# kwea123/nerf_pl

Measured on AMD Instinct MI355X. Metric: rays/sec (64+128 samples), full training step: render_rays fwd + MSE + bwd + grad all-reduce + Adam, higher is better.
Workload: dtype bf16

## Files before the change

include/nerfhip.h:

```cpp
#ifndef NERFHIP_H
#define NERFHIP_H

#include <stddef.h>
#include <stdint.h>

#ifdef __cplusplus
extern "C" {
#endif

#define NERFHIP_ABI_VERSION 3

#define NERFHIP_E_BADARG (-1)
#define NERFHIP_E_UNSUPPORTED (-2)
#define NERFHIP_E_ALIGN (-3)
#define NERFHIP_E_DATA (-4)

#define NERFHIP_F32 0
#define NERFHIP_BF16 1
#define NERFHIP_BF16_F8 2

typedef void* nerfhip_stream_t;

int nerfhip_abi_version(void);
const char* nerfhip_error_string(int code);

int nerfhip_posenc(const float* x, float* out, int64_t n, int C, int n_freqs, nerfhip_stream_t stream);
int nerfhip_posenc_bwd(const float* x, const float* gout, float* gx, int64_t n, int C, int n_freqs,
                       nerfhip_stream_t stream);

int nerfhip_posenc_bands(const float* x, const float* bands, float* out, int64_t n, int C, int n_freqs,
                         nerfhip_stream_t stream);
int nerfhip_posenc_bands_bwd(const float* x, const float* bands, const float* gout, float* gx, int64_t n, int C, int n_freqs,
                             nerfhip_stream_t stream);

int nerfhip_sample_coarse_z(const float* rays, const float* perturb_rand, float* z, int64_t B, int S,
                            int use_disp, float perturb, nerfhip_stream_t stream);

int nerfhip_searchsorted_right(const float* a, const float* v, int64_t* idx, int64_t B, int M, int K,
                               nerfhip_stream_t stream);
int nerfhip_searchsorted_left(const float* a, const float* v, int64_t* idx, int64_t B, int M, int K,
                              nerfhip_stream_t stream);

int nerfhip_sample_pdf(const float* bins, int64_t bins_stride, const float* weights, int64_t w_stride,
                       const float* u, int64_t u_stride, float* samples, int64_t B, int M, int K, float eps,
                       nerfhip_stream_t stream);

#define NERFHIP_ROW_TOTAL_EXACT 0
#define NERFHIP_ROW_TOTAL_ATEN 1

int nerfhip_sample_pdf_ex(const float* bins, int64_t bins_stride, const float* weights, int64_t w_stride,
                          const float* u, int64_t u_stride, float* samples, int64_t B, int M, int K, float eps,
                          float* cdf_out, int64_t* inds_out, int row_total, nerfhip_stream_t stream);

int nerfhip_fine_z(const float* z_coarse, const float* w_coarse, const float* u, int64_t u_stride,
                   float* z_fine, float* z_new, int64_t B, int S_c, int N_i, float eps,
                   nerfhip_stream_t stream);

int nerfhip_fine_z_ex(const float* z_coarse, const float* w_coarse, const float* u, int64_t u_stride, float* z_fine,
                      float* z_new, int64_t B, int S_c, int N_i, float eps, float* cdf_out, int64_t* inds_out,
                      int row_total, nerfhip_stream_t stream);

int nerfhip_composite_fwd(const float* raw, int raw_ch, const float* z, const float* rays,
                          const float* noise, float noise_std, int white_back, float* weights, float* rgb,
                          float* depth, float* opacity, int64_t B, int S, nerfhip_stream_t stream);
int nerfhip_composite_bwd(const float* raw, int raw_ch, const float* z, const float* rays,
                          const float* noise, float noise_std, int white_back, const float* g_rgb,
                          const float* g_depth, const float* g_opacity, const float* g_weights,
                          float* g_raw, int64_t B, int S, nerfhip_stream_t stream);

int nerfhip_composite_train(const float* raw, const float* z, const float* rays, const float* noise, float noise_std,
                            int white_back, const float* target, float grad_scale, float* weights, float* rgb, float* depth,
                            float* opacity, float* g_raw, int64_t B, int S, nerfhip_stream_t stream);

int nerfhip_composite_train_fine_z(const float* raw, const float* z, const float* rays, const float* noise, float noise_std,
                                   int white_back, const float* target, float grad_scale, float* weights, float* rgb, float* depth,
                                   float* opacity, float* g_raw, int64_t B, int S, const float* u, int64_t u_stride, int N_i,
                                   float eps, float* z_fine, int row_total, nerfhip_stream_t stream);
int nerfhip_composite_train_loss(const float* raw, const float* z, const float* rays, const float* noise, float noise_std,
                                 int white_back, const float* target, float grad_scale, float* weights, float* rgb, float* depth,
                                 float* opacity, float* g_raw, int64_t B, int S, const float* rgb_coarse, float* out3,
                                 uint32_t* ticket, nerfhip_stream_t stream);

size_t nerfhip_mlp_packed_bytes(int dtype);
int nerfhip_mlp_pack_weights(const float* const* weights_host, const float* const* biases_host, void* packed,
                             int dtype, nerfhip_stream_t stream);

size_t nerfhip_mlp_act_bytes(int64_t n_points, int dtype);

int nerfhip_mlp_fwd_embedded(const float* x, int64_t x_stride, int64_t n, const void* packed, float* out,
                             int sigma_only, int dtype, void* save_acts, nerfhip_stream_t stream);

int nerfhip_mlp_fwd_rays(const float* rays, const float* z, int64_t B, int S, const void* packed, float* out,
                         int sigma_only, int dtype, void* save_acts, nerfhip_stream_t stream);

int nerfhip_mlp_fwd_rays_coarse(const float* rays, const float* perturb_rand, float* z, int64_t B, int S, int use_disp,
                                float perturb, const void* packed, float* out, int sigma_only, int dtype, void* save_acts,
                                nerfhip_stream_t stream);

size_t nerfhip_mlp_packed_bwd_bytes(int dtype);
int nerfhip_mlp_pack_weights_bwd(const float* const* weights_host, const float* const* biases_host, void* packed_bwd, int dtype,
                                 nerfhip_stream_t stream);
int nerfhip_mlp_pack_weights_train(const float* const* weights_host, const float* const* biases_host, void* packed,
                                   void* packed_bwd, int dtype, nerfhip_stream_t stream);
int nerfhip_mlp_pack_weights_train_multi(const float* const* weights_host, const float* const* biases_host,
                                         void* const* packed_host, void* const* packed_bwd_host, int n_models, int dtype,
                                         nerfhip_stream_t stream);
size_t nerfhip_mlp_dy_bytes(int64_t n_points, int dtype);
int nerfhip_mlp_dw_splits(int64_t n_points, int dtype);
size_t nerfhip_mlp_dw_workspace_bytes(int64_t n_points, int dtype);
int nerfhip_mlp_bwd(const float* g_out, const float* out, int64_t n, const void* packed_bwd, const void* acts,
                    void* dys, void* dw_workspace, float* const* grad_w_host, float* const* grad_b_host,
                    int accumulate, int dtype, nerfhip_stream_t stream);

int nerfhip_mlp_bwd_phases(const float* g_out, const float* out, int64_t n, const void* packed_bwd, const void* acts,
                           void* dys, void* dw_workspace, float* const* grad_w_host, float* const* grad_b_host,
                           int accumulate, int dtype, int phases, nerfhip_stream_t stream);

typedef struct nerfhip_adam_fused {
    int n_models;
    float* param[2];
    float* exp_avg[2];
    float* exp_avg_sq[2];
    const float* grad_flat[2];
    float* state;
    float lr, beta1, beta2, eps, weight_decay;
} nerfhip_adam_fused;
size_t nerfhip_mlp_dw_workspace_bytes_multi(const int64_t* n_points_host, int n_models, int dtype);
int nerfhip_mlp_dw_plan(const int64_t* n_points_host, int n_models, int dtype, int* splits_out, int* stage_kib_out);
int nerfhip_mlp_bwd_multi(int n_models, const float* const* g_out_host, const float* const* out_host, const int64_t* n_host,
                          const void* const* packed_bwd_host, const void* const* acts_host, void* const* dys_host,
                          void* dw_workspace, float* const* grad_w_host, float* const* grad_b_host, int accumulate, int dtype,
                          int phases, const float* g_scale, const nerfhip_adam_fused* adam, nerfhip_stream_t stream);

typedef struct nerfhip_enc_source {
    const float* rays[2];
    const float* z[2];
    int S[2];
} nerfhip_enc_source;
int nerfhip_mlp_bwd_multi_rays(int n_models, const float* const* g_out_host, const float* const* out_host, const int64_t* n_host,
                               const void* const* packed_bwd_host, const void* const* acts_host, void* const* dys_host,
                               void* dw_workspace, float* const* grad_w_host, float* const* grad_b_host, int accumulate, int dtype,
                               int phases, const float* g_scale, const nerfhip_adam_fused* adam, const nerfhip_enc_source* enc,
                               nerfhip_stream_t stream);

int nerfhip_mlp_dx_embedded(const void* dys, int64_t n, const float* w_xyz1, const float* w_xyz5, const float* w_dir,
                            float* gx, int64_t gx_stride, int dtype, nerfhip_stream_t stream);

#define NERFHIP_ACT_NONE 0
#define NERFHIP_ACT_RELU 1
#define NERFHIP_ACT_SIGMOID 2
int nerfhip_linear_fwd(const float* x, int64_t ldx, const float* w, int64_t ldw, const float* bias, float* y, int64_t ldy,
                       int64_t n, int n_in, int n_out, int act, int accumulate, int dtype, nerfhip_stream_t stream);
int nerfhip_linear_bwd_input(const float* gy, int64_t ldgy, const float* y, int64_t ldy, int act, const float* w, int64_t ldw,
                             float* gx, int64_t ldgx, int64_t n, int n_in, int n_out, int accumulate, int dtype,
                             nerfhip_stream_t stream);
size_t nerfhip_linear_bwd_weight_workspace_bytes(int64_t n, int n_in, int n_out);
int nerfhip_linear_bwd_weight(const float* gy, int64_t ldgy, const float* y, int64_t ldy, int act, const float* x, int64_t ldx,
                              float* gw, int64_t ldgw, float* gb, void* workspace, int64_t n, int n_in, int n_out,
                              int accumulate, int dtype, nerfhip_stream_t stream);

int nerfhip_mse_psnr(const float* rgb_coarse, const float* rgb_fine, const float* target, int64_t n, float* out3,
                     float* g_coarse, float* g_fine, nerfhip_stream_t stream);

int nerfhip_adam_step(float* const* params_host, const float* const* grads_host, float* const* exp_avg_host,
                      float* const* exp_avg_sq_host, const int64_t* numel_host, int n_tensors, float* state, float lr,
                      float beta1, float beta2, float eps, float weight_decay, nerfhip_stream_t stream);

int nerfhip_radam_step(float* const* params_host, const float* const* grads_host, float* const* exp_avg_host,
                       float* const* exp_avg_sq_host, const int64_t* numel_host, int n_tensors, float* state, double lr,
                       double beta1, double beta2, double eps, double weight_decay, int degenerated_to_sgd,
                       nerfhip_stream_t stream);
int nerfhip_ranger_step(float* const* params_host, const float* const* grads_host, float* const* exp_avg_host,
                        float* const* exp_avg_sq_host, const int64_t* numel_host, int n_tensors, float* state,
                        float* const* slow_host, double alpha, int k, double n_sma_threshold, double lr, double beta1,
                        double beta2, double eps, double weight_decay, nerfhip_stream_t stream);

int nerfhip_ray_directions(float* dirs, int H, int W, double focal, nerfhip_stream_t stream);
int nerfhip_get_rays(const float* directions, const float* c2w, float* rays_o, float* rays_d, int64_t n,
                     nerfhip_stream_t stream);
int nerfhip_ndc_rays(int H, int W, double focal, float near, const float* rays_o, const float* rays_d, float* out_o,
                     float* out_d, int64_t n, nerfhip_stream_t stream);
int nerfhip_gen_rays(const float* c2w, const int64_t* pixel_ids, int64_t first_pixel, int64_t n, int H, int W,
                     double focal, float near, float far, int use_ndc, float ndc_near_plane, float* rays,
                     nerfhip_stream_t stream);
int nerfhip_sample_batch(const float* c2w, const int64_t* pixel_ids, const float* rgbs_all, int64_t n, int H, int W,
                         double focal, float near, float far, int use_ndc, float ndc_near_plane, float* rays, float* rgbs,
                         nerfhip_stream_t stream);

#define NERFHIP_DRAW_UNIFORM 0
#define NERFHIP_DRAW_NORMAL 1
#define NERFHIP_DRAW_RANDINT 2
typedef struct nerfhip_draw {
    int kind;
    int64_t numel;
    void* out;
    uint64_t range;
} nerfhip_draw;
typedef struct nerfhip_ray_batch {
    const float* c2w;
    const float* rgbs_all;
    float* rays;
    float* rgbs;
    int H, W;
    double focal;
    float near, far;
    int use_ndc;
    float ndc_near_plane;
} nerfhip_ray_batch;
uint64_t nerfhip_torch_draw_increment(int64_t numel, int max_blocks);
int nerfhip_torch_draws(const nerfhip_draw* draws_host, int n_draws, const nerfhip_ray_batch* batch_host, uint64_t seed,
                        uint64_t offset, uint64_t* state, int max_blocks, uint64_t* increment_host, nerfhip_stream_t stream);

int nerfhip_train_prologue(const nerfhip_draw* draws_host, int n_draws, const nerfhip_ray_batch* batch_host, uint64_t seed,
                           uint64_t offset, uint64_t* state, int max_blocks, uint64_t* increment_host,
                           const float* const* weights_host, const float* const* biases_host, void* const* packed_host,
                           void* const* packed_bwd_host, int n_models, int dtype, nerfhip_stream_t stream);

typedef struct nerfhip_render_args {
    const float* rays;
    int64_t B;
    int S_c, N_i;
    const void* packed_coarse;
    const void* packed_fine;
    float* z_coarse;
    float* raw_coarse;
    float* z_fine;
    float* raw_fine;
    void* save_coarse;
    void* save_fine;
    const float* perturb_rand;
    float perturb;
    int use_disp;
    const float* noise_coarse;
    const float* noise_fine;
    float noise_std;
    int white_back;
    const float* u;
    int64_t u_stride;
    float eps;
    int row_total;
    float* rgb_coarse;
    float* depth_coarse;
    float* opacity_coarse;
    float* rgb_fine;
    float* depth_fine;
    float* opacity_fine;
    const float* target;
    float grad_scale;
    float* g_raw_coarse;
    float* g_raw_fine;
    float* out3;
    uint32_t* ticket;
    int regen_enc;
} nerfhip_render_args;
int nerfhip_render_supported(int64_t B, int S_c, int N_i, int dtype);
int nerfhip_render_fwd(const nerfhip_render_args* args_host, int dtype, nerfhip_stream_t stream);
int nerfhip_render_test_fwd(const nerfhip_render_args* args_host, int dtype, nerfhip_stream_t stream);
int nerfhip_render_train_fwd(const nerfhip_render_args* args_host, int dtype, nerfhip_stream_t stream);

size_t nerfhip_marching_cubes_workspace_bytes(int64_t n0, int64_t n1, int64_t n2);
int nerfhip_marching_cubes_count(const float* volume, int64_t n0, int64_t n1, int64_t n2, double iso, void* workspace,
                                 int64_t* totals, nerfhip_stream_t stream);
int nerfhip_marching_cubes_emit(const float* volume, int64_t n0, int64_t n1, int64_t n2, double iso, void* workspace,
                                const int64_t* totals, double* vertices, int32_t* triangles, nerfhip_stream_t stream);

int nerfhip_mesh_edge_keys(const int32_t* triangles, int64_t T, int64_t* keys, nerfhip_stream_t stream);
size_t nerfhip_mesh_cluster_workspace_bytes(int64_t V, int64_t T);
int nerfhip_mesh_largest_cluster(const int32_t* triangles, int64_t V, int64_t T, const int64_t* sorted_keys, const int64_t* order,
                                 void* workspace, int64_t* totals, nerfhip_stream_t stream);
int nerfhip_mesh_cluster_compact(const int32_t* triangles, int64_t V, int64_t T, void* workspace, int64_t* kept_vertex_ids,
                                 int32_t* kept_triangles, nerfhip_stream_t stream);

int nerfhip_mesh_vertex_normals(const float* vertices, int64_t V, const int32_t* triangles, int64_t T, double* normals,
                                nerfhip_stream_t stream);
int nerfhip_mesh_normal_rays(const float* vertices, const double* normals, int64_t V, float near, float far, float near_t,
                             float* rays, nerfhip_stream_t stream);
int nerfhip_mesh_view_rays(const float* vertices, int64_t V, const float* w2c_host, const float* origin_host, float focal, int W,
                           int H, const uint8_t* image, float near, uint8_t* colors, double* depth, float* rays,
                           nerfhip_stream_t stream);
int nerfhip_mesh_color_accumulate(const uint8_t* colors, const double* depth, const float* opacity, int64_t V,
                                  float occ_threshold, double* accum, nerfhip_stream_t stream);
int nerfhip_mesh_color_finish(const double* accum, int64_t V, uint8_t* out, nerfhip_stream_t stream);
int nerfhip_mesh_rgb_to_u8(const float* rgb, int64_t n, uint8_t* out, nerfhip_stream_t stream);

size_t nerfhip_vol_workspace_bytes(int64_t n);
int nerfhip_vol_pack(const float* rgbsigma, int64_t n, int64_t first_index, float neg_cell, void* workspace, uint32_t* records,
                     int64_t capacity, int64_t* cursor, nerfhip_stream_t stream);

int nerfhip_png_unfilter(const uint8_t* streams, uint8_t* out, int32_t* error_flags, int n_images, int H, int W, int ch,
                         nerfhip_stream_t stream);
int nerfhip_resize_rgba_lanczos(const uint8_t* in, uint8_t* out, uint8_t* workspace, int n_images, int in_h, int in_w, int out_h,
                                int out_w, const int32_t* xmin_h, const int32_t* count_h, const int32_t* taps_h, int ksize_h,
                                const int32_t* xmin_v, const int32_t* count_v, const int32_t* taps_v, int ksize_v,
                                nerfhip_stream_t stream);
int nerfhip_rgba_to_rgb_white(const uint8_t* rgba, float* rgb, uint8_t* valid_mask, int64_t n, nerfhip_stream_t stream);

int nerfhip_jpeg_entropy_decode(const uint8_t* scan, int64_t scan_bytes, int n_comp, const int32_t* comp, const uint8_t* huffman,
                                int huffman_mask, int mcus_x, int mcus_y, int restart_interval, int16_t* const* coef,
                                const int64_t* coef_blocks);
size_t nerfhip_jpeg_planes_bytes(int H, int W, int n_comp, int hs, int vs);
int nerfhip_jpeg_decode(const int16_t* coef_y, const int16_t* coef_cb, const int16_t* coef_cr, const uint16_t* quant,
                        uint8_t* planes, uint8_t* out, int n_images, int H, int W, int n_comp, int hs, int vs,
                        nerfhip_stream_t stream);

#define NERFHIP_IMAGE_PLANAR 0
#define NERFHIP_IMAGE_INTERLEAVED 1
size_t nerfhip_ssim_workspace_bytes(int B, int C, int H, int W);
int nerfhip_ssim(const float* img1, const float* img2, int B, int C, int H, int W, int window_size, int layout, float* map,
                 float* mean, void* workspace, nerfhip_stream_t stream);
size_t nerfhip_depth_colormap_workspace_bytes(int64_t n);
int nerfhip_depth_colormap(const float* depth, int64_t n, const uint8_t* table, float* out_chw, uint8_t* out_hwc, void* workspace,
                           nerfhip_stream_t stream);

#define NERFHIP_GIF_STRIP 3838
size_t nerfhip_gif_workspace_bytes(int F, int H, int W);
size_t nerfhip_gif_data_stride(int H, int W);
int nerfhip_gif_quantize(const uint8_t* frames, int F, int H, int W, uint8_t* indices, uint8_t* palettes, int32_t* box_counts,
                         void* workspace, nerfhip_stream_t stream);
int nerfhip_gif_lzw(const uint8_t* indices, int F, int H, int W, uint8_t* data, int32_t* lengths, void* workspace,
                    nerfhip_stream_t stream);

#ifdef __cplusplus
}
#endif
#endif
```

nerf_pl_amd/_lib.py:

```python
import ctypes
import functools
import os

import torch

_PKG = os.path.dirname(os.path.abspath(__file__))
LIB_PATH = os.environ.get("NERFHIP_LIB_PATH") or os.path.join(_PKG, "libnerfhip.so")

F32, BF16, BF16_F8 = 0, 1, 2

_c_void_p = ctypes.c_void_p
_i64 = ctypes.c_int64
_int = ctypes.c_int
_f32 = ctypes.c_float
_f64 = ctypes.c_double

SIGNATURES = {
    "nerfhip_abi_version": [],
    "nerfhip_error_string": [_int],
    "nerfhip_posenc": [_c_void_p, _c_void_p, _i64, _int, _int, _c_void_p],
    "nerfhip_posenc_bwd": [_c_void_p, _c_void_p, _c_void_p, _i64, _int, _int, _c_void_p],
    "nerfhip_posenc_bands": [_c_void_p, _c_void_p, _c_void_p, _i64, _int, _int, _c_void_p],
    "nerfhip_posenc_bands_bwd": [_c_void_p, _c_void_p, _c_void_p, _c_void_p, _i64, _int, _int, _c_void_p],
    "nerfhip_sample_coarse_z": [_c_void_p, _c_void_p, _c_void_p, _i64, _int, _int, _f32, _c_void_p],
    "nerfhip_searchsorted_right": [_c_void_p, _c_void_p, _c_void_p, _i64, _int, _int, _c_void_p],
    "nerfhip_searchsorted_left": [_c_void_p, _c_void_p, _c_void_p, _i64, _int, _int, _c_void_p],
    "nerfhip_sample_pdf": [_c_void_p, _i64, _c_void_p, _i64, _c_void_p, _i64, _c_void_p, _i64, _int, _int, _f32,
                           _c_void_p],
    "nerfhip_sample_pdf_ex": [_c_void_p, _i64, _c_void_p, _i64, _c_void_p, _i64, _c_void_p, _i64, _int, _int, _f32,
                              _c_void_p, _c_void_p, _int, _c_void_p],
    "nerfhip_fine_z_ex": [_c_void_p, _c_void_p, _c_void_p, _i64, _c_void_p, _c_void_p, _i64, _int, _int, _f32,
                          _c_void_p, _c_void_p, _int, _c_void_p],
    "nerfhip_fine_z": [_c_void_p, _c_void_p, _c_void_p, _i64, _c_void_p, _c_void_p, _i64, _int, _int, _f32,
                       _c_void_p],
    "nerfhip_composite_fwd": [_c_void_p, _int, _c_void_p, _c_void_p, _c_void_p, _f32, _int, _c_void_p, _c_void_p,
                              _c_void_p, _c_void_p, _i64, _int, _c_void_p],
    "nerfhip_composite_bwd": [_c_void_p, _int, _c_void_p, _c_void_p, _c_void_p, _f32, _int, _c_void_p, _c_void_p,
                              _c_void_p, _c_void_p, _c_void_p, _i64, _int, _c_void_p],
    "nerfhip_mlp_packed_bytes": [_int],
    "nerfhip_mlp_pack_weights": [ctypes.POINTER(_c_void_p), ctypes.POINTER(_c_void_p), _c_void_p, _int, _c_void_p],
    "nerfhip_mlp_act_bytes": [_i64, _int],
    "nerfhip_mlp_fwd_embedded": [_c_void_p, _i64, _i64, _c_void_p, _c_void_p, _int, _int, _c_void_p, _c_void_p],
    "nerfhip_mlp_fwd_rays": [_c_void_p, _c_void_p, _i64, _int, _c_void_p, _c_void_p, _int, _int, _c_void_p, _c_void_p],
    "nerfhip_mlp_packed_bwd_bytes": [_int],
    "nerfhip_mlp_pack_weights_bwd": [ctypes.POINTER(_c_void_p), ctypes.POINTER(_c_void_p), _c_void_p, _int, _c_void_p],
    "nerfhip_mlp_pack_weights_train": [ctypes.POINTER(_c_void_p), ctypes.POINTER(_c_void_p), _c_void_p, _c_void_p, _int, _c_void_p],
    "nerfhip_mlp_dy_bytes": [_i64, _int],
    "nerfhip_mlp_dw_splits": [_i64, _int],
    "nerfhip_mlp_dw_workspace_bytes": [_i64, _int],
    "nerfhip_ray_directions": [_c_void_p, _int, _int, ctypes.c_double, _c_void_p],
    "nerfhip_get_rays": [_c_void_p, _c_void_p, _c_void_p, _c_void_p, _i64, _c_void_p],
    "nerfhip_ndc_rays": [_int, _int, ctypes.c_double, _f32, _c_void_p, _c_void_p, _c_void_p, _c_void_p, _i64, _c_void_p],
    "nerfhip_gen_rays": [_c_void_p, _c_void_p, _i64, _i64, _int, _int, ctypes.c_double, _f32, _f32, _int, _f32, _c_void_p,
                         _c_void_p],
    "nerfhip_mse_psnr": [_c_void_p, _c_void_p, _c_void_p, _i64, _c_void_p, _c_void_p, _c_void_p, _c_void_p],
    "nerfhip_mlp_bwd_phases": [_c_void_p, _c_void_p, _i64, _c_void_p, _c_void_p, _c_void_p, _c_void_p,
                               ctypes.POINTER(_c_void_p), ctypes.POINTER(_c_void_p), _int, _int, _int, _c_void_p],
    "nerfhip_mlp_dx_embedded": [_c_void_p, _i64, _c_void_p, _c_void_p, _c_void_p, _c_void_p, _i64, _int, _c_void_p],
    "nerfhip_adam_step": [ctypes.POINTER(_c_void_p), ctypes.POINTER(_c_void_p), ctypes.POINTER(_c_void_p),
                          ctypes.POINTER(_c_void_p), ctypes.POINTER(_i64), _int, _c_void_p, _f32, _f32, _f32, _f32, _f32, _c_void_p],
    "nerfhip_radam_step": [ctypes.POINTER(_c_void_p), ctypes.POINTER(_c_void_p), ctypes.POINTER(_c_void_p),
                           ctypes.POINTER(_c_void_p), ctypes.POINTER(_i64), _int, _c_void_p, _f64, _f64, _f64, _f64, _f64, _int, _c_void_p],
    "nerfhip_ranger_step": [ctypes.POINTER(_c_void_p), ctypes.POINTER(_c_void_p), ctypes.POINTER(_c_void_p),
                            ctypes.POINTER(_c_void_p), ctypes.POINTER(_i64), _int, _c_void_p, ctypes.POINTER(_c_void_p), _f64, _int,
                            _f64, _f64, _f64, _f64, _f64, _f64, _c_void_p],
    "nerfhip_mlp_bwd": [_c_void_p, _c_void_p, _i64, _c_void_p, _c_void_p, _c_void_p, _c_void_p,
                        ctypes.POINTER(_c_void_p), ctypes.POINTER(_c_void_p), _int, _int, _c_void_p],
    "nerfhip_sample_batch": [_c_void_p, _c_void_p, _c_void_p, _i64, _int, _int, ctypes.c_double, _f32, _f32, _int, _f32, _c_void_p,
                             _c_void_p, _c_void_p],
    "nerfhip_mlp_pack_weights_train_multi": [ctypes.POINTER(_c_void_p), ctypes.POINTER(_c_void_p), ctypes.POINTER(_c_void_p),
                                             ctypes.POINTER(_c_void_p), _int, _int, _c_void_p],
    "nerfhip_render_supported": [_i64, _int, _int, _int],
    "nerfhip_render_test_fwd": [_c_void_p, _int, _c_void_p],
    "nerfhip_render_fwd": [_c_void_p, _int, _c_void_p],
    "nerfhip_render_train_fwd": [_c_void_p, _int, _c_void_p],
    "nerfhip_composite_train": [_c_void_p, _c_void_p, _c_void_p, _c_void_p, _f32, _int, _c_void_p, _f32, _c_void_p, _c_void_p,
                                _c_void_p, _c_void_p, _c_void_p, _i64, _int, _c_void_p],
    "nerfhip_composite_train_fine_z": [_c_void_p, _c_void_p, _c_void_p, _c_void_p, _f32, _int, _c_void_p, _f32, _c_void_p, _c_void_p,
                                       _c_void_p, _c_void_p, _c_void_p, _i64, _int, _c_void_p, _i64, _int, _f32, _c_void_p, _int, _c_void_p],
    "nerfhip_composite_train_loss": [_c_void_p, _c_void_p, _c_void_p, _c_void_p, _f32, _int, _c_void_p, _f32, _c_void_p, _c_void_p,
                                     _c_void_p, _c_void_p, _c_void_p, _i64, _int, _c_void_p, _c_void_p, _c_void_p, _c_void_p],
    "nerfhip_mlp_fwd_rays_coarse": [_c_void_p, _c_void_p, _c_void_p, _i64, _int, _int, _f32, _c_void_p, _c_void_p, _int, _int,
                                    _c_void_p, _c_void_p],
    "nerfhip_torch_draw_increment": [_i64, _int],
    "nerfhip_torch_draws": [_c_void_p, _int, _c_void_p, ctypes.c_uint64, ctypes.c_uint64, _c_void_p, _int,
                            ctypes.POINTER(ctypes.c_uint64), _c_void_p],
    "nerfhip_train_prologue": [_c_void_p, _int, _c_void_p, ctypes.c_uint64, ctypes.c_uint64, _c_void_p, _int,
                               ctypes.POINTER(ctypes.c_uint64), ctypes.POINTER(_c_void_p), ctypes.POINTER(_c_void_p),
                               ctypes.POINTER(_c_void_p), ctypes.POINTER(_c_void_p), _int, _int, _c_void_p],
    "nerfhip_mlp_dw_workspace_bytes_multi": [ctypes.POINTER(_i64), _int, _int],
    "nerfhip_mlp_dw_plan": [ctypes.POINTER(_i64), _int, _int, ctypes.POINTER(_int), ctypes.POINTER(_int)],
    "nerfhip_mlp_bwd_multi": [_int, ctypes.POINTER(_c_void_p), ctypes.POINTER(_c_void_p), ctypes.POINTER(_i64),
                              ctypes.POINTER(_c_void_p), ctypes.POINTER(_c_void_p), ctypes.POINTER(_c_void_p), _c_void_p,
                              ctypes.POINTER(_c_void_p), ctypes.POINTER(_c_void_p), _int, _int, _int, _c_void_p, _c_void_p, _c_void_p],
    "nerfhip_mlp_bwd_multi_rays": [_int, ctypes.POINTER(_c_void_p), ctypes.POINTER(_c_void_p), ctypes.POINTER(_i64),
                                   ctypes.POINTER(_c_void_p), ctypes.POINTER(_c_void_p), ctypes.POINTER(_c_void_p), _c_void_p,
                                   ctypes.POINTER(_c_void_p), ctypes.POINTER(_c_void_p), _int, _int, _int, _c_void_p, _c_void_p, _c_void_p,
                                   _c_void_p],
    "nerfhip_linear_fwd": [_c_void_p, _i64, _c_void_p, _i64, _c_void_p, _c_void_p, _i64, _i64, _int, _int, _int, _int, _int, _c_void_p],
    "nerfhip_linear_bwd_input": [_c_void_p, _i64, _c_void_p, _i64, _int, _c_void_p, _i64, _c_void_p, _i64, _i64, _int, _int, _int,
                                 _int, _c_void_p],
    "nerfhip_linear_bwd_weight_workspace_bytes": [_i64, _int, _int],
    "nerfhip_linear_bwd_weight": [_c_void_p, _i64, _c_void_p, _i64, _int, _c_void_p, _i64, _c_void_p, _i64, _c_void_p, _c_void_p,
                                  _i64, _int, _int, _int, _int, _c_void_p],
    "nerfhip_marching_cubes_workspace_bytes": [_i64, _i64, _i64],
    "nerfhip_marching_cubes_count": [_c_void_p, _i64, _i64, _i64, ctypes.c_double, _c_void_p, _c_void_p, _c_void_p],
    "nerfhip_marching_cubes_emit": [_c_void_p, _i64, _i64, _i64, ctypes.c_double, _c_void_p, _c_void_p, _c_void_p, _c_void_p,
                                    _c_void_p],
    "nerfhip_mesh_edge_keys": [_c_void_p, _i64, _c_void_p, _c_void_p],
    "nerfhip_mesh_cluster_workspace_bytes": [_i64, _i64],
    "nerfhip_mesh_largest_cluster": [_c_void_p, _i64, _i64, _c_void_p, _c_void_p, _c_void_p, _c_void_p, _c_void_p],
    "nerfhip_mesh_cluster_compact": [_c_void_p, _i64, _i64, _c_void_p, _c_void_p, _c_void_p, _c_void_p],
    "nerfhip_mesh_vertex_normals": [_c_void_p, _i64, _c_void_p, _i64, _c_void_p, _c_void_p],
    "nerfhip_mesh_normal_rays": [_c_void_p, _c_void_p, _i64, _f32, _f32, _f32, _c_void_p, _c_void_p],
    "nerfhip_mesh_view_rays": [_c_void_p, _i64, ctypes.POINTER(_f32), ctypes.POINTER(_f32), _f32, _int, _int, _c_void_p, _f32,
                               _c_void_p, _c_void_p, _c_void_p, _c_void_p],
    "nerfhip_mesh_color_accumulate": [_c_void_p, _c_void_p, _c_void_p, _i64, _f32, _c_void_p, _c_void_p],
    "nerfhip_mesh_color_finish": [_c_void_p, _i64, _c_void_p, _c_void_p],
    "nerfhip_mesh_rgb_to_u8": [_c_void_p, _i64, _c_void_p, _c_void_p],
    "nerfhip_vol_workspace_bytes": [_i64],
    "nerfhip_vol_pack": [_c_void_p, _i64, _i64, _f32, _c_void_p, _c_void_p, _i64, _c_void_p, _c_void_p],
    "nerfhip_png_unfilter": [_c_void_p, _c_void_p, _c_void_p, _int, _int, _int, _int, _c_void_p],
    "nerfhip_resize_rgba_lanczos": [_c_void_p, _c_void_p, _c_void_p, _int, _int, _int, _int, _int, _c_void_p, _c_void_p, _c_void_p,
                                    _int, _c_void_p, _c_void_p, _c_void_p, _int, _c_void_p],
    "nerfhip_rgba_to_rgb_white": [_c_void_p, _c_void_p, _c_void_p, _i64, _c_void_p],
    "nerfhip_jpeg_entropy_decode": [_c_void_p, _i64, _int, _c_void_p, _c_void_p, _int, _int, _int, _int, ctypes.POINTER(_c_void_p),
                                    ctypes.POINTER(_i64)],
    "nerfhip_jpeg_planes_bytes": [_int, _int, _int, _int, _int],
    "nerfhip_jpeg_decode": [_c_void_p, _c_void_p, _c_void_p, _c_void_p, _c_void_p, _c_void_p, _int, _int, _int, _int, _int, _int,
                            _c_void_p],
    "nerfhip_ssim_workspace_bytes": [_int, _int, _int, _int],
    "nerfhip_ssim": [_c_void_p, _c_void_p, _int, _int, _int, _int, _int, _int, _c_void_p, _c_void_p, _c_void_p, _c_void_p],
    "nerfhip_depth_colormap_workspace_bytes": [_i64],
    "nerfhip_depth_colormap": [_c_void_p, _i64, _c_void_p, _c_void_p, _c_void_p, _c_void_p, _c_void_p],
    "nerfhip_gif_workspace_bytes": [_int, _int, _int],
    "nerfhip_gif_data_stride": [_int, _int],
    "nerfhip_gif_quantize": [_c_void_p, _int, _int, _int, _c_void_p, _c_void_p, _c_void_p, _c_void_p, _c_void_p],
    "nerfhip_gif_lzw": [_c_void_p, _int, _int, _int, _c_void_p, _c_void_p, _c_void_p, _c_void_p],
}


class AdamFused(ctypes.Structure):
    _fields_ = [("n_models", _int), ("param", _c_void_p * 2), ("exp_avg", _c_void_p * 2), ("exp_avg_sq", _c_void_p * 2),
                ("grad_flat", _c_void_p * 2), ("state", _c_void_p), ("lr", _f32), ("beta1", _f32), ("beta2", _f32), ("eps", _f32),
                ("weight_decay", _f32)]

class Draw(ctypes.Structure):
    _fields_ = [("kind", _int), ("numel", _i64), ("out", _c_void_p), ("range", ctypes.c_uint64)]


class RayBatch(ctypes.Structure):
    _fields_ = [("c2w", _c_void_p), ("rgbs_all", _c_void_p), ("rays", _c_void_p), ("rgbs", _c_void_p), ("H", _int), ("W", _int),
                ("focal", ctypes.c_double), ("near", _f32), ("far", _f32), ("use_ndc", _int), ("ndc_near_plane", _f32)]


class RenderArgs(ctypes.Structure):
    _fields_ = [("rays", _c_void_p), ("B", _i64), ("S_c", _int), ("N_i", _int), ("packed_coarse", _c_void_p), ("packed_fine", _c_void_p),
                ("z_coarse", _c_void_p), ("raw_coarse", _c_void_p), ("z_fine", _c_void_p), ("raw_fine", _c_void_p),
                ("save_coarse", _c_void_p), ("save_fine", _c_void_p), ("perturb_rand", _c_void_p), ("perturb", _f32), ("use_disp", _int),
                ("noise_coarse", _c_void_p), ("noise_fine", _c_void_p), ("noise_std", _f32), ("white_back", _int), ("u", _c_void_p),
                ("u_stride", _i64), ("eps", _f32), ("row_total", _int), ("rgb_coarse", _c_void_p), ("depth_coarse", _c_void_p),
                ("opacity_coarse", _c_void_p), ("rgb_fine", _c_void_p), ("depth_fine", _c_void_p), ("opacity_fine", _c_void_p),
                ("target", _c_void_p), ("grad_scale", _f32), ("g_raw_coarse", _c_void_p), ("g_raw_fine", _c_void_p), ("out3", _c_void_p),
                ("ticket", _c_void_p), ("regen_enc", _int)]


class EncSource(ctypes.Structure):
    _fields_ = [("rays", _c_void_p * 2), ("z", _c_void_p * 2), ("S", _int * 2)]


DRAW_UNIFORM, DRAW_NORMAL, DRAW_RANDINT = 0, 1, 2

_RESTYPES = {"nerfhip_error_string": ctypes.c_char_p, "nerfhip_torch_draw_increment": ctypes.c_uint64, "nerfhip_mlp_packed_bytes": ctypes.c_size_t,
             "nerfhip_mlp_act_bytes": ctypes.c_size_t, "nerfhip_mlp_packed_bwd_bytes": ctypes.c_size_t,
             "nerfhip_mlp_dy_bytes": ctypes.c_size_t, "nerfhip_mlp_dw_workspace_bytes": ctypes.c_size_t,
             "nerfhip_mlp_dw_workspace_bytes_multi": ctypes.c_size_t,
             "nerfhip_linear_bwd_weight_workspace_bytes": ctypes.c_size_t,
             "nerfhip_marching_cubes_workspace_bytes": ctypes.c_size_t, "nerfhip_mesh_cluster_workspace_bytes": ctypes.c_size_t,
             "nerfhip_jpeg_planes_bytes": ctypes.c_size_t, "nerfhip_ssim_workspace_bytes": ctypes.c_size_t,
             "nerfhip_depth_colormap_workspace_bytes": ctypes.c_size_t, "nerfhip_gif_workspace_bytes": ctypes.c_size_t,
             "nerfhip_gif_data_stride": ctypes.c_size_t, "nerfhip_vol_workspace_bytes": ctypes.c_size_t}

_lib = None


class NerfHipError(RuntimeError):
    pass


def load():
    global _lib
    if _lib is not None:
        return _lib
    if not os.path.exists(LIB_PATH):
        raise NerfHipError(
            "libnerfhip.so not built: run `python -m nerf_pl_amd.build` (needs hipcc, gfx950). "
            "There is no CPU/eager fallback for the hot path.")
    lib = ctypes.CDLL(LIB_PATH, mode=ctypes.RTLD_GLOBAL)
    for name, argtypes in SIGNATURES.items():
        fn = getattr(lib, name)
        fn.argtypes = argtypes
        fn.restype = _RESTYPES.get(name, ctypes.c_int)
    if lib.nerfhip_abi_version() != 3:
        raise NerfHipError("libnerfhip ABI version mismatch")
    _lib = lib
    return lib


def check(code, what):
    if code != 0:
        msg = load().nerfhip_error_string(code)
        raise NerfHipError("%s failed: %s (code %d)" % (what, msg.decode() if msg else "?", code))


def stream_ptr():
    return ctypes.c_void_p(torch.cuda.current_stream().cuda_stream)


def _first_cuda_tensor(args):
    for a in args:
        if torch.is_tensor(a) and a.is_cuda:
            return a
        if isinstance(a, (list, tuple)):
            t = _first_cuda_tensor(a)
            if t is not None:
                return t
    return None


def device_guard(fn):
    @functools.wraps(fn)
    def wrapped(*args, **kw):
        t = _first_cuda_tensor(args)
        if t is None:
            t = _first_cuda_tensor(tuple(kw.values()))
        if t is None or t.device.index == torch.cuda.current_device():
            return fn(*args, **kw)
        with torch.cuda.device(t.device):
            return fn(*args, **kw)
    return wrapped


def ptr(t):
    if t is None:
        return None
    return ctypes.c_void_p(t.data_ptr())


def require_gpu(*tensors):
    dev = None
    for t in tensors:
        if t is None:
            continue
        if not t.is_cuda:
            raise NerfHipError("nerf_pl_amd runs on MI355X only: got a %s tensor (no CPU fallback)" % t.device)
        if t.dtype != torch.float32:
            raise NerfHipError("expected float32 tensor, got %s" % t.dtype)
        if dev is None:
            dev = t.device
        elif t.device != dev:
            raise NerfHipError("tensors of one call live on different GPUs (%s vs %s)" % (dev, t.device))
    if dev is not None and dev.index != torch.cuda.current_device():
        raise NerfHipError("launch on %s while the current device is cuda:%d (operator missing its device_guard)"
                           % (dev, torch.cuda.current_device()))
```

nerf_pl_amd/csrc/mlp_bwd.hip:

```cpp
#include "common.h"
#include "mlp_layout.h"
#include "mlp_bwd_chain.h"
#include "mlp_bwd_dw.h"
#include "mlp_dw_plan.h"

static_assert(kPlanF32 == NERFHIP_F32 && kPlanBf16 == NERFHIP_BF16 && kPlanBf16F8 == NERFHIP_BF16_F8, "mlp_dw_plan.h dtype codes");
static inline bool valid_dtype(int dtype) { return dtype == NERFHIP_F32 || dtype == NERFHIP_BF16 || dtype == NERFHIP_BF16_F8; }
static inline int compute_prec(int dtype) { return dtype == NERFHIP_F32 ? NERFHIP_F32 : NERFHIP_BF16; }
#if NERFHIP_DW_PROBE
static bool g_probe_f8 = false;
#endif

extern "C" size_t nerfhip_mlp_dy_bytes(int64_t n_points, int dtype) {
    if (n_points < 0 || !valid_dtype(dtype)) return 0;
    if (dtype == NERFHIP_BF16_F8) return (size_t)act_tiles(n_points, dtype) * nerfhip::mlp::f8_dy_tile_bytes();
    return (size_t)act_tiles(n_points, dtype) * nerfhip::mlp::kDySlabs * 64 * (dtype == NERFHIP_BF16 ? 16 : 32);
}

extern "C" int nerfhip_mlp_dw_splits(int64_t n_points, int dtype) {
    if (n_points <= 0 || !valid_dtype(dtype)) return 0;
    return dw_plan(&n_points, 1, dtype, nullptr);
}
static size_t dw_workspace_bytes(int nwg, int n_models) {
    return ((size_t)nwg * nerfhip::mlp::kDwSlabFloats + (size_t)n_models * nerfhip::mlp::kFoldScratchFloats) * sizeof(float);
}
extern "C" size_t nerfhip_mlp_dw_workspace_bytes(int64_t n_points, int dtype) {
    const int nwg = nerfhip_mlp_dw_splits(n_points, dtype);
    return nwg > 0 ? dw_workspace_bytes(nwg, 1) : 0;
}
extern "C" size_t nerfhip_mlp_dw_workspace_bytes_multi(const int64_t* n_points_host, int n_models, int dtype) {
    if (!n_points_host || n_models < 1 || n_models > nerfhip::kDwMaxModels || !valid_dtype(dtype)) return 0;
    for (int m = 0; m < n_models; ++m)
        if (n_points_host[m] <= 0) return 0;
    return dw_workspace_bytes(dw_plan(n_points_host, n_models, dtype, nullptr), n_models);
}

extern "C" int nerfhip_mlp_dw_plan(const int64_t* n_points_host, int n_models, int dtype, int* splits_out, int* stage_kib_out) {
    if (!n_points_host || !splits_out || n_models < 1 || n_models > nerfhip::kDwMaxModels || !valid_dtype(dtype)) return NERFHIP_E_BADARG;
    for (int m = 0; m < n_models; ++m)
        if (n_points_host[m] <= 0) return NERFHIP_E_BADARG;
    nerfhip::DwJobTable jt;
    const int total = dw_plan(n_points_host, n_models, dtype, &jt);
    for (int j = 0; j < n_models * nerfhip::mlp::kNumDwJobs; ++j) {
        splits_out[j] = jt.nsplit[j];
        if (stage_kib_out) {
            int slabs = jt.job[j].dy_slabs + jt.job[j].x1_slabs + jt.job[j].x2_slabs;
            if (jt.fold_of[j] >= 0 || jt.nsplit[j] == 0) slabs = 0;
            for (int k = 0; k < n_models * nerfhip::mlp::kNumDwJobs; ++k)
                if (jt.fold_of[k] == j) slabs += jt.job[k].dy_slabs;
            stage_kib_out[j] = dtype == NERFHIP_F32 ? 2 * slabs : slabs;
        }
    }
    return total;
}

extern "C" int nerfhip_mlp_bwd_multi(int n_models, const float* const* g_out_host, const float* const* out_host,
                                     const int64_t* n_host, const void* const* packed_bwd_host, const void* const* acts_host,
                                     void* const* dys_host, void* dw_workspace, float* const* grad_w_host,
                                     float* const* grad_b_host, int accumulate, int dtype, int phases, const float* g_scale,
                                     const nerfhip_adam_fused* adam, nerfhip_stream_t stream) {
    return nerfhip_mlp_bwd_multi_rays(n_models, g_out_host, out_host, n_host, packed_bwd_host, acts_host, dys_host, dw_workspace, grad_w_host,
                                      grad_b_host, accumulate, dtype, phases, g_scale, adam, nullptr, stream);
}

extern "C" int nerfhip_mlp_bwd_multi_rays(int n_models, const float* const* g_out_host, const float* const* out_host,
                                          const int64_t* n_host, const void* const* packed_bwd_host, const void* const* acts_host,
                                          void* const* dys_host, void* dw_workspace, float* const* grad_w_host,
                                          float* const* grad_b_host, int accumulate, int dtype, int phases, const float* g_scale,
                                          const nerfhip_adam_fused* adam, const nerfhip_enc_source* enc, nerfhip_stream_t stream) {
    NERFHIP_CHECK_ARG(n_models >= 1 && n_models <= nerfhip::kDwMaxModels);
    if (!valid_dtype(dtype)) return NERFHIP_E_UNSUPPORTED;
    bool regen[nerfhip::kDwMaxModels] = {false, false};
    if (enc) {
        if (dtype != NERFHIP_BF16) return NERFHIP_E_UNSUPPORTED;
        for (int m = 0; m < n_models; ++m) {
            if (!enc->rays[m]) continue;
            NERFHIP_CHECK_ARG(enc->z[m] && enc->S[m] > 0 && enc->S[m] % 32 == 0 && n_host[m] % 256 == 0 && n_host[m] % enc->S[m] == 0);
            NERFHIP_CHECK_ARG(n_host[m] / 32 < (int64_t)1 << 31);
            if ((((uintptr_t)enc->rays[m]) | ((uintptr_t)enc->z[m])) & 15) return NERFHIP_E_ALIGN;
            regen[m] = true;
        }
    }
    NERFHIP_CHECK_ARG(g_out_host && out_host && n_host && packed_bwd_host && acts_host && dys_host && grad_w_host && grad_b_host);
    NERFHIP_CHECK_ARG(!(adam && accumulate));
    nerfhip::GradTable G;
    nerfhip::DwJobTable jt;
    for (int m = 0; m < n_models; ++m) {
        NERFHIP_CHECK_ARG(n_host[m] > 0);
        NERFHIP_CHECK_ARG(g_out_host[m] && out_host[m] && packed_bwd_host[m] && acts_host[m] && dys_host[m] && dw_workspace);
        if ((((uintptr_t)g_out_host[m]) | ((uintptr_t)out_host[m]) | ((uintptr_t)packed_bwd_host[m]) | ((uintptr_t)acts_host[m]) |
             ((uintptr_t)dys_host[m])) & 15)
            return NERFHIP_E_ALIGN;
    }
    const int nwg = dw_plan(n_host, n_models, dtype, &jt);
    for (int m = 0; m < nerfhip::kDwMaxModels; ++m) {
        const bool on = m < n_models && regen[m];
        jt.enc_rays[m] = on ? enc->rays[m] : nullptr;
        jt.enc_z[m] = on ? enc->z[m] : nullptr;
        jt.enc_tpr[m] = on ? enc->S[m] / 32 : 1;
    }
    float* const fold_scratch = (float*)dw_workspace + (size_t)nwg * nerfhip::mlp::kDwSlabFloats;
    nerfhip::FoldArgs F;
    for (int m = 0; m < nerfhip::kDwMaxModels; ++m) {
        const int mm = m < n_models ? m : 0;
        F.image[m] = reinterpret_cast<const float*>((const uint8_t*)packed_bwd_host[mm] +
                                                    (size_t)nerfhip::mlp::bwd_padded_pieces(compute_prec(dtype)) * nerfhip::mlp::kPieceBytes);
        F.gw_final[m] = grad_w_host[12 * mm + 8];
        F.gb_final[m] = grad_b_host[12 * mm + 8];
        F.gw_dir[m] = grad_w_host[12 * mm + 9];
    }
    for (int j = 0; j < nerfhip::kDwMaxJobs; ++j) {
        const int jj = j < jt.njobs ? j : 0, m = jj / nerfhip::mlp::kNumDwJobs, prm = nerfhip::mlp::kDwJobs[jj % nerfhip::mlp::kNumDwJobs].param;
        NERFHIP_CHECK_ARG(grad_w_host[12 * m + prm] && grad_b_host[12 * m + prm]);
        G.w[j] = grad_w_host[12 * m + prm];
        G.b[j] = grad_b_host[12 * m + prm];
        jt.acts[j] = (const uint8_t*)acts_host[m];
        jt.dys[j] = (const uint8_t*)dys_host[m];
    }
    nerfhip::AdamFused A;
    A.state = nullptr;
    A.lr = A.beta1 = A.beta2 = A.eps = A.wd = 0.f;
    for (int m = 0; m < nerfhip::kDwMaxModels; ++m) { A.param[m] = A.m[m] = A.v[m] = nullptr; A.grad0[m] = nullptr; }
    if (adam) {
        NERFHIP_CHECK_ARG(adam->state && adam->n_models == n_models);
        for (int m = 0; m < n_models; ++m) {
            NERFHIP_CHECK_ARG(adam->param[m] && adam->exp_avg[m] && adam->exp_avg_sq[m] && adam->grad_flat[m]);
            A.param[m] = adam->param[m]; A.m[m] = adam->exp_avg[m]; A.v[m] = adam->exp_avg_sq[m]; A.grad0[m] = adam->grad_flat[m];
        }
        A.state = adam->state; A.lr = adam->lr; A.beta1 = adam->beta1; A.beta2 = adam->beta2; A.eps = adam->eps; A.wd = adam->weight_decay;
    }
    hipStream_t s = (hipStream_t)stream;
    const bool do_chain = phases & 1, do_dw = phases & 2, do_reduce = phases & 4;
    if (do_chain) {
        int64_t tiles[nerfhip::kDwMaxModels];
        for (int m = 0; m < n_models; ++m) tiles[m] = act_tiles(n_host[m], dtype);
        nerfhip::launch_bwd_chain(n_models, g_out_host, g_scale, out_host, n_host, packed_bwd_host, acts_host, dys_host, dtype, tiles, s);
    }
    if (do_dw) {
        if (dtype == NERFHIP_BF16_F8) nerfhip::launch_dw_f8(jt, (float*)dw_workspace, nwg, s);
        else nerfhip::launch_dw(dtype, jt, (float*)dw_workspace, nwg, s);
#if NERFHIP_DW_PROBE
        g_probe_f8 = dtype == NERFHIP_BF16_F8;
#endif
    }
    if (do_reduce) {
        nerfhip::launch_reduce(dtype == NERFHIP_BF16_F8, jt, (const float*)dw_workspace, G, fold_scratch, accumulate, A, s);
        nerfhip::launch_fold(F, (const float*)fold_scratch, n_models, accumulate, A, s);
    }
    return nerfhip_launch_status();
}

#if NERFHIP_DW_PROBE
extern "C" int nerfhip_debug_dw_probe(unsigned* host_dst, int n_words) {
    if (!host_dst || n_words < 0 || n_words > 1024 * 8 * 8) return NERFHIP_E_BADARG;
    return g_probe_f8 ? nerfhip::read_dw_f8_probe(host_dst, n_words) : nerfhip::read_dw_probe(host_dst, n_words);
}
#endif

extern "C" int nerfhip_mlp_bwd_phases(const float* g_out, const float* out, int64_t n, const void* packed_bwd, const void* acts,
                                      void* dys, void* dw_workspace, float* const* grad_w_host, float* const* grad_b_host,
                                      int accumulate, int dtype, int phases, nerfhip_stream_t stream) {
    NERFHIP_CHECK_ARG(n >= 0);
    if (!valid_dtype(dtype)) return NERFHIP_E_UNSUPPORTED;
    NERFHIP_CHECK_ARG(grad_w_host && grad_b_host);
    for (int i = 0; i < 12; ++i) NERFHIP_CHECK_ARG(grad_w_host[i] && grad_b_host[i]);
    if (n == 0) return 0;
    return nerfhip_mlp_bwd_multi(1, &g_out, &out, &n, &packed_bwd, &acts, &dys, dw_workspace, grad_w_host, grad_b_host, accumulate,
                                 dtype, phases, nullptr, nullptr, stream);
}

extern "C" int nerfhip_mlp_bwd(const float* g_out, const float* out, int64_t n, const void* packed_bwd, const void* acts,
                               void* dys, void* dw_workspace, float* const* grad_w_host, float* const* grad_b_host,
                               int accumulate, int dtype, nerfhip_stream_t stream) {
    return nerfhip_mlp_bwd_phases(g_out, out, n, packed_bwd, acts, dys, dw_workspace, grad_w_host, grad_b_host, accumulate, dtype, 7,
                                  stream);
}
```

nerf_pl_amd/csrc/mlp_bwd_dw.h:

```cpp
#pragma once
#include <stdint.h>

#include "mlp_layout.h"

typedef struct ihipStream_t* hipStream_t;

#ifndef NERFHIP_DW_PROBE
#define NERFHIP_DW_PROBE 0
#endif

namespace nerfhip {
using namespace mlp;

constexpr int kDwMaxModels = 2;
constexpr int kDwMaxJobs = kDwMaxModels * kNumDwJobs;
struct DwJobTable {
    DwJob job[kDwMaxJobs];
    int nsplit[kDwMaxJobs];
    int soff[kDwMaxJobs + 1];
    const uint8_t* acts[kDwMaxJobs];
    const uint8_t* dys[kDwMaxJobs];
    int64_t ntiles[kDwMaxJobs];
    int njobs;
    int fold_of[kDwMaxJobs];
    const float* enc_rays[kDwMaxModels];
    const float* enc_z[kDwMaxModels];
    int enc_tpr[kDwMaxModels];
};
static_assert(kDwJobs[kDwJobDir].x2_off == kDwJobs[kDwJobSigma].x1_off && kDwJobs[kDwJobDir].x2_slabs == 16 && kDwJobs[kDwJobDir].x1_slabs == 2 &&
              kDwJobs[kDwJobSigma].x1_slabs == 16 && kDwJobs[kDwJobSigma].dy_slabs == 2 && kDwJobs[kDwJobDir].dy_slabs == 8 &&
              kDwJobs[kDwJobSigma].x2_slabs == 0, "the sigma head and the dir layer read the same h8 section");
constexpr int kDwFoldRow0 = 4;
NH_HD constexpr int dw_fold_block(int xt) { return (kDwFoldRow0 + xt / 2) * kDwMaxXTiles + (xt & 1); }
constexpr int kDwFoldStageSlabs = 28;
constexpr int kDwFoldSigmaSlab = 26;

struct GradTable {
    float* w[kDwMaxJobs];
    float* b[kDwMaxJobs];
};

struct AdamFused {
    float* param[kDwMaxModels];
    float* m[kDwMaxModels];
    float* v[kDwMaxModels];
    const float* grad0[kDwMaxModels];
    float* state;
    float lr, beta1, beta2, eps, wd;
};

struct FoldArgs {
    const float* image[kDwMaxModels];
    float* gw_final[kDwMaxModels];
    float* gb_final[kDwMaxModels];
    float* gw_dir[kDwMaxModels];
};

void launch_dw(int prec, const DwJobTable& jt, float* slabs, int nwg, hipStream_t s);
void launch_dw_f8(const DwJobTable& jt, float* slabs, int nwg, hipStream_t s);
void launch_reduce(bool f8, const DwJobTable& jt, const float* slabs, const GradTable& G, float* fold_scratch, int accumulate,
                   const AdamFused& A, hipStream_t s);
void launch_fold(const FoldArgs& F, const float* fold_scratch, int n_models, int accumulate, const AdamFused& A, hipStream_t s);
#if NERFHIP_DW_PROBE
int read_dw_probe(unsigned* host_dst, int n_words);
int read_dw_f8_probe(unsigned* host_dst, int n_words);
#endif
}
```

nerf_pl_amd/csrc/mlp_bwd_reduce.hip:

```cpp
#include "mlp_device.h"
#include "adam_math.h"
#include "mlp_bwd_dw.h"

namespace nerfhip {

struct GradEmit {
    const AdamFused& A;
    AdamCoef ac;
    int accumulate, model;
    __device__ __forceinline__ void operator()(float* dst, float val) const {
        const float g = accumulate ? *dst + val : val;
        *dst = g;
        if (A.state) {
            const size_t e = (size_t)(dst - A.grad0[model]);
            adam_elem(A.param[model][e], g, A.m[model][e], A.v[model][e], ac, A.beta2, A.eps, A.wd);
        }
    }
};

template <bool F8>
__global__ __launch_bounds__(256) void mlp_bwd_reduce_kernel(DwJobTable jobs, const float* __restrict__ slabs, GradTable G,
                                                              float* __restrict__ fold_scratch, int accumulate, AdamFused A) {
    const int jid = blockIdx.y;
    const DwJob jb = jobs.job[jid];
    const int model = jid / kNumDwJobs;
    const int fold = jobs.fold_of[jid];
    const int nsplit = jobs.nsplit[fold >= 0 ? fold : jid], s0 = jobs.soff[fold >= 0 ? fold : jid];
    const bool derived = jid % kNumDwJobs == kDwJobFinal;
    const int n_ot = derived ? 0 : jb.dy_slabs / 2, n_xt = (jb.x1_slabs + jb.x2_slabs) / 2;
    float* const scratch = fold_scratch + (size_t)model * kFoldScratchFloats;
    const int n_out = kParamOut[jb.param], ldw = kParamIn[jb.param];
    const int tile = blockIdx.x;
    const int ot = tile / (kDwMaxXTiles + 1), xt = tile % (kDwMaxXTiles + 1);
    AdamCoef ac;
    if (A.state) ac = adam_coef(A.state[0] + 1.0f, A.lr, A.beta1, A.beta2);
    const GradEmit emit{A, ac, accumulate, model};
    if (ot < n_ot && xt == kDwMaxXTiles) {
        const int m = threadIdx.x;
        if (m < 32) {
            float sacc = 0.f;
            for (int sp = 0; sp < nsplit; ++sp) {
                const float* sl = slabs + (size_t)(s0 + sp) * kDwSlabFloats + (size_t)8 * kDwMaxXTiles * 64 * 16 +
                                  (fold >= 0 ? kDwFoldRow0 : ot) * 64;
                sacc += F8 ? sl[m] : sl[m] + sl[m + 32];
            }
            const int o = F8 ? 32 * ot + chain_feature(m >> 4, f8_row_h(m & 15), f8_row_j(m & 15)) : 32 * ot + m;
            if (o < n_out) {
                emit(G.b[jid] + o, sacc);
                if (jid % kNumDwJobs == kDwJobDir) scratch[kFoldS + o] = sacc;
            }
        }
    } else if (ot < n_ot && xt < n_xt) {
        const int e4 = threadIdx.x;
        const float4* src = reinterpret_cast<const float4*>(slabs + (size_t)s0 * kDwSlabFloats +
                                                            ((size_t)(fold >= 0 ? dw_fold_block(xt) : ot * kDwMaxXTiles + xt) * 64) * 16) + e4;
        float4 acc = make_float4(0.f, 0.f, 0.f, 0.f);
#pragma unroll 8
        for (int sp = 0; sp < nsplit; ++sp) {
            const float4 v = src[(size_t)sp * (kDwSlabFloats / 4)];
            acc.x += v.x; acc.y += v.y; acc.z += v.z; acc.w += v.w;
        }
        const int lane = e4 & 63, rq = e4 >> 6;
        const int h = lane >> 5, ncol = lane & 31;
        const int m0 = 8 * rq + 4 * h;
        const int o0 = F8 ? 32 * ot + chain_feature(m0 >> 4, f8_row_h(m0 & 15), f8_row_j(m0 & 15)) : 32 * ot + m0;
        const int xi = 32 * xt + ncol;
        int xs = xi >> 4;
        const int i = xi & 15;
        const int sh = F8 ? f8_row_h(i) : slab_nat_h(i), sj = F8 ? f8_row_j(i) : slab_nat_j(i);
        int enc, col0;
        if (xs < jb.x1_slabs) { enc = jb.x1_enc; col0 = jb.x1_col0; }
        else { xs -= jb.x1_slabs; enc = jb.x2_enc; col0 = jb.x2_col0; }
        int col;
        if (enc == 0 || enc == kDwEncFold) col = col0 + chain_feature(xs, sh, sj);
        else {
            const int ch = (enc == 1) ? xyz_slot_channel(xs, sh, sj) : dir_slot_channel(xs, sh, sj);
            col = ch < 0 ? -1 : col0 + ch;
        }
        if (enc == kDwEncFold) {
            const float vals[4] = {acc.x, acc.y, acc.z, acc.w};
#pragma unroll
            for (int k = 0; k < 4; ++k)
                if (o0 + k < n_out) scratch[kFoldG + (size_t)(o0 + k) * kW + col] = vals[k];
        } else if (col >= 0 && col < ldw) {
            const float vals[4] = {acc.x, acc.y, acc.z, acc.w};
#pragma unroll
            for (int k = 0; k < 4; ++k) {
                const int o = o0 + k;
                if (o < n_out) emit(G.w[jid] + (size_t)o * ldw + col, vals[k]);
            }
        }
    }
    if (A.state) {
        __syncthreads();
        if (threadIdx.x == 0) {
            unsigned* ticket = reinterpret_cast<unsigned*>(A.state + 1);
            const unsigned prev = atomicAdd(ticket, 1u);
            if (prev == gridDim.x * gridDim.y - 1) {
                *ticket = 0u;
                A.state[0] = A.state[0] + 1.0f;
            }
        }
    }
}

constexpr int kFoldBlocks = 32 + 64 + 1;
__global__ __launch_bounds__(256) void mlp_bwd_fold_kernel(FoldArgs F, const float* __restrict__ fold_scratch, int accumulate, AdamFused A) {
    constexpr int PA = 257, PB = 33;
    __shared__ float lds[2 * 32 * PA];
    __shared__ float part[4][16][64];
    const int model = blockIdx.y, bx = blockIdx.x, t = threadIdx.x;
    const int lane = t & 63, wave = t >> 6;
    const float* __restrict__ Gm = fold_scratch + (size_t)model * kFoldScratchFloats + kFoldG;
    const float* __restrict__ sv = fold_scratch + (size_t)model * kFoldScratchFloats + kFoldS;
    const float* __restrict__ Wf = F.image[model] + (size_t)kFoldWf * 256;
    const float* __restrict__ Wdx = F.image[model] + (size_t)kFoldWdx * 256;
    const float* __restrict__ bf = F.image[model] + (size_t)kFoldBf * 256;
    AdamCoef ac;
    if (A.state) ac = adam_coef(A.state[0], A.lr, A.beta1, A.beta2);
    const GradEmit emit{A, ac, accumulate, model};
    if (bx == kFoldBlocks - 1) {
        float a4[4] = {0.f, 0.f, 0.f, 0.f};
#pragma unroll 8
        for (int j = 0; j < 128; j += 4)
#pragma unroll
            for (int q = 0; q < 4; ++q) a4[q] = __builtin_fmaf(Wdx[(size_t)(j + q) * 256 + t], sv[j + q], a4[q]);
        emit(F.gb_final[model] + t, (a4[0] + a4[1]) + (a4[2] + a4[3]));
        return;
    }
    const bool dir = bx < 32;
    const int row0 = dir ? 32 * (bx >> 3) : 32 * ((bx - 32) >> 3), col0 = dir ? 32 * (bx & 7) : 32 * ((bx - 32) & 7);
    f32x16 acc;
#pragma unroll
    for (int r = 0; r < 16; ++r) acc[r] = 0.0f;
    const int m = lane & 31, kh = lane >> 5;
    if (dir) {
        float* sa = lds;
        float* sb = lds + 32 * PA;
        float4 va[8], vb[8];
#pragma unroll
        for (int i = 0; i < 8; ++i) {
            const int row = (t >> 6) + 4 * i;
            va[i] = reinterpret_cast<const float4*>(Gm + (size_t)(row0 + row) * 256)[t & 63];
            vb[i] = reinterpret_cast<const float4*>(Wf + (size_t)(col0 + row) * 256)[t & 63];
        }
#pragma unroll
        for (int i = 0; i < 8; ++i) {
            const int o = ((t >> 6) + 4 * i) * PA + 4 * (t & 63);
            sa[o] = va[i].x; sa[o + 1] = va[i].y; sa[o + 2] = va[i].z; sa[o + 3] = va[i].w;
            sb[o] = vb[i].x; sb[o + 1] = vb[i].y; sb[o + 2] = vb[i].z; sb[o + 3] = vb[i].w;
        }
        __syncthreads();
        const float* pa = sa + m * PA + 64 * wave + kh;
        const float* pb = sb + m * PA + 64 * wave + kh;
#pragma unroll 8
        for (int k = 0; k < 64; k += 2) acc = __builtin_amdgcn_mfma_f32_32x32x2f32(pa[k], pb[k], acc, 0, 0, 0);
    } else {
        float* sa = lds;
        float* sb = lds + 128 * PB;
        const int c = t & 31, r0 = t >> 5;
        float va[16], vb[16];
#pragma unroll
        for (int i = 0; i < 16; ++i) {
            va[i] = Wdx[(size_t)(r0 + 8 * i) * 256 + row0 + c];
            vb[i] = Gm[(size_t)(r0 + 8 * i) * 256 + col0 + c];
        }
#pragma unroll
        for (int i = 0; i < 16; ++i) {
            sa[(r0 + 8 * i) * PB + c] = va[i];
            sb[(r0 + 8 * i) * PB + c] = vb[i];
        }
        __syncthreads();
        const float* pa = sa + (32 * wave + kh) * PB + m;
        const float* pb = sb + (32 * wave + kh) * PB + m;
#pragma unroll 8
        for (int j = 0; j < 32; j += 2) acc = __builtin_amdgcn_mfma_f32_32x32x2f32(pa[j * PB], pb[j * PB], acc, 0, 0, 0);
    }
#pragma unroll
    for (int r = 0; r < 16; ++r) part[wave][r][lane] = acc[r];
    __syncthreads();
#pragma unroll
    for (int i = 0; i < 4; ++i) {
        const int r = wave + 4 * i;
        const float v = ((part[0][r][lane] + part[1][r][lane]) + part[2][r][lane]) + part[3][r][lane];
        const int row = row0 + (r & 3) + 8 * (r >> 2) + 4 * (lane >> 5), col = col0 + (lane & 31);
        if (dir) emit(F.gw_dir[model] + (size_t)row * kParamIn[9] + col, __builtin_fmaf(sv[row], bf[col], v));
        else emit(F.gw_final[model] + (size_t)row * 256 + col, v);
    }
}

void launch_reduce(bool f8, const DwJobTable& jt, const float* slabs, const GradTable& G, float* fold_scratch, int accumulate,
                   const AdamFused& A, hipStream_t s) {
    const dim3 rgrid(8 * (kDwMaxXTiles + 1), (unsigned)jt.njobs);
    if (f8) hipLaunchKernelGGL(mlp_bwd_reduce_kernel<true>, rgrid, dim3(256), 0, s, jt, slabs, G, fold_scratch, accumulate, A);
    else hipLaunchKernelGGL(mlp_bwd_reduce_kernel<false>, rgrid, dim3(256), 0, s, jt, slabs, G, fold_scratch, accumulate, A);
}
void launch_fold(const FoldArgs& F, const float* fold_scratch, int n_models, int accumulate, const AdamFused& A, hipStream_t s) {
    hipLaunchKernelGGL(mlp_bwd_fold_kernel, dim3(kFoldBlocks, (unsigned)n_models), dim3(256), 0, s, F, fold_scratch, accumulate, A);
}

}
```

nerf_pl_amd/csrc/mlp_render.hip:

```cpp
#include "common.h"
#include "mlp_layout.h"

namespace nerfhip {
using namespace mlp;
typedef nerfhip_render_args RenderArgs;
constexpr int kRenderRays = 4;

template <int PREC, int SV>
int launch_render_variant(const RenderArgs& a, unsigned groups, hipStream_t stream);
template <> int launch_render_variant<NERFHIP_F32, 0>(const RenderArgs&, unsigned, hipStream_t);
template <> int launch_render_variant<NERFHIP_F32, 1>(const RenderArgs&, unsigned, hipStream_t);
template <> int launch_render_variant<NERFHIP_BF16, 0>(const RenderArgs&, unsigned, hipStream_t);
template <> int launch_render_variant<NERFHIP_BF16, 1>(const RenderArgs&, unsigned, hipStream_t);
template <> int launch_render_variant<NERFHIP_BF16, 2>(const RenderArgs&, unsigned, hipStream_t);
template <> int launch_render_variant<NERFHIP_F32, 3>(const RenderArgs&, unsigned, hipStream_t);
template <> int launch_render_variant<NERFHIP_BF16, 3>(const RenderArgs&, unsigned, hipStream_t);

static int render_tail_floats_host(int S_c, int N_i) {
    const int S_f = S_c + N_i;
    const int S4 = (S_c + 3) & ~3, N4 = (N_i + 3) & ~3, F4 = (S_f + 3) & ~3;
    const int fz = N_i > 0 ? 3 * S4 + N4 + ((S_c + 1 + 3) & ~3) + N4 : 0;
    const int coarse = 2 * S4 + fz;
    return coarse > F4 ? coarse : F4;
}

static bool render_shape_ok(int64_t B, int S_c, int N_i, int dtype) {
    if (dtype != NERFHIP_F32 && dtype != NERFHIP_BF16 && dtype != NERFHIP_BF16_F8) return false;
    const int pts = 32 * (dtype == NERFHIP_F32 ? 4 : 8);
    if (B <= 0 || B % kRenderRays != 0 || B / kRenderRays > 0x7fffffff || S_c < 3 || N_i < 0) return false;
    if ((kRenderRays * S_c) % pts != 0 || (N_i > 0 && (kRenderRays * (S_c + N_i)) % pts != 0)) return false;
    if ((int64_t)B * (S_c + N_i) / pts > 0x7fffffff) return false;
    return (size_t)kRenderRays * render_tail_floats_host(S_c, N_i) * sizeof(float) <= (size_t)kSlots * kChunkBytes;
}

static int render_check(const RenderArgs* a, int dtype, bool train) {
    NERFHIP_CHECK_ARG(a != nullptr);
    if (!render_shape_ok(a->B, a->S_c, a->N_i, dtype)) return NERFHIP_E_UNSUPPORTED;
    const bool fine = a->N_i > 0;
    NERFHIP_CHECK_ARG(a->rays && a->packed_coarse && a->z_coarse && a->raw_coarse && a->opacity_coarse);
    NERFHIP_CHECK_ARG(!fine || (a->packed_fine && a->z_fine && a->raw_fine && a->rgb_fine && a->depth_fine && a->opacity_fine));
    NERFHIP_CHECK_ARG(a->perturb <= 0.0f || a->perturb_rand);
    NERFHIP_CHECK_ARG(a->noise_std == 0.0f || (a->noise_coarse && (!fine || a->noise_fine)));
    NERFHIP_CHECK_ARG(a->row_total == NERFHIP_ROW_TOTAL_EXACT || a->row_total == NERFHIP_ROW_TOTAL_ATEN);
    if (train)
        NERFHIP_CHECK_ARG(a->target && a->rgb_coarse && a->depth_coarse && a->g_raw_coarse && a->save_coarse && a->out3 && a->ticket &&
                          (!fine || (a->g_raw_fine && a->save_fine)));
    uintptr_t lines = (uintptr_t)a->z_coarse | (uintptr_t)a->raw_coarse | (uintptr_t)a->z_fine | (uintptr_t)a->raw_fine;
    if (train) lines |= (uintptr_t)a->g_raw_coarse | (uintptr_t)a->g_raw_fine;
    if ((lines & 127) || (((uintptr_t)a->packed_coarse | (uintptr_t)a->packed_fine) & 15)) return NERFHIP_E_ALIGN;
    return 0;
}

}

extern "C" int nerfhip_render_supported(int64_t B, int S_c, int N_i, int dtype) {
    return nerfhip::render_shape_ok(B, S_c, N_i, dtype) ? 1 : 0;
}

extern "C" int nerfhip_render_fwd(const nerfhip_render_args* args, int dtype, nerfhip_stream_t stream) {
    using namespace nerfhip;
    if (args && args->B == 0) return 0;
    const int rc = render_check(args, dtype, false);
    if (rc) return rc;
    const unsigned groups = (unsigned)(args->B / kRenderRays);
    if (dtype == NERFHIP_F32) return launch_render_variant<NERFHIP_F32, 0>(*args, groups, (hipStream_t)stream);
    return launch_render_variant<NERFHIP_BF16, 0>(*args, groups, (hipStream_t)stream);
}

extern "C" int nerfhip_render_test_fwd(const nerfhip_render_args* args, int dtype, nerfhip_stream_t stream) {
    using namespace nerfhip;
    if (args && args->B == 0) return 0;
    const int rc = render_check(args, dtype, false);
    if (rc) return rc;
    NERFHIP_CHECK_ARG(args->N_i > 0);
    const unsigned groups = (unsigned)(args->B / kRenderRays);
    if (dtype == NERFHIP_F32) return launch_render_variant<NERFHIP_F32, 3>(*args, groups, (hipStream_t)stream);
    return launch_render_variant<NERFHIP_BF16, 3>(*args, groups, (hipStream_t)stream);
}

extern "C" int nerfhip_render_train_fwd(const nerfhip_render_args* args, int dtype, nerfhip_stream_t stream) {
    using namespace nerfhip;
    if (args && args->B == 0) return 0;
    const int rc = render_check(args, dtype, true);
    if (rc) return rc;
    const unsigned groups = (unsigned)(args->B / kRenderRays);
    if (dtype == NERFHIP_F32) return launch_render_variant<NERFHIP_F32, 1>(*args, groups, (hipStream_t)stream);
    if (dtype == NERFHIP_BF16_F8) return launch_render_variant<NERFHIP_BF16, 2>(*args, groups, (hipStream_t)stream);
    return launch_render_variant<NERFHIP_BF16, 1>(*args, groups, (hipStream_t)stream);
}
```

nerf_pl_amd/csrc/mlp_render_kernel.h:

```cpp
#pragma once
#include "composite_wave.h"
#include "mlp_fwd_kernel.h"

namespace nerfhip {

constexpr int kRenderRays = 4;

typedef nerfhip_render_args RenderArgs;

__host__ __device__ inline int render_tail_floats(int S_c, int N_i, int S_f) {
    const int S4 = (S_c + 3) & ~3, N4 = (N_i + 3) & ~3, F4 = (S_f + 3) & ~3;
    const int fz = N_i > 0 ? 3 * S4 + N4 + ((S_c + 1 + 3) & ~3) + N4 : 0;
    const int coarse = 2 * S4 + fz;
    return coarse > F4 ? coarse : F4;
}

__device__ __forceinline__ void render_wg_sync() {
    asm volatile("s_waitcnt vmcnt(0) lgkmcnt(0)\n\ts_barrier" ::: "memory");
}

typedef const RenderArgs __attribute__((address_space(4)))* RenderArgsP;
__device__ __forceinline__ RenderArgsP render_args() {
    RenderArgsP p = (RenderArgsP)__builtin_amdgcn_kernarg_segment_ptr();
    asm volatile("" : "+s"(p));
    return p;
}

template <bool TRAIN, int NW, bool TT = false>
__device__ __forceinline__ void render_tail(const bool fine_pass, const bool with_fine_z, float* const tail_lds, const int wave,
                                            const int lane) {
    constexpr int R = kRenderRays;
    const RenderArgsP a = render_args();
    const int S_c = a->S_c, N_i = a->N_i, S_f = S_c + N_i;
    const float noise_std = a->noise_std;
    const float* raw = fine_pass ? a->raw_fine : a->raw_coarse;
    const float* z = fine_pass ? a->z_fine : a->z_coarse;
    const float* noise = noise_std != 0.0f ? (fine_pass ? a->noise_fine : a->noise_coarse) : nullptr;
    const int S = fine_pass ? S_f : S_c;
    float* rgb = fine_pass ? a->rgb_fine : a->rgb_coarse;
    float* depth = fine_pass ? a->depth_fine : a->depth_coarse;
    float* opac = fine_pass ? a->opacity_fine : a->opacity_coarse;
    const float* rays = a->rays;
    const int white_back = a->white_back;
    const int per_ray = render_tail_floats(S_c, N_i, S_f);
    const int S4 = (S_c + 3) & ~3;
    const int64_t ray0 = (int64_t)blockIdx.x * R, B = a->B;
    const int njobs = with_fine_z ? 2 * R : R;
    for (int job = wave; job < njobs; job += NW) {
        const int slot = job < R ? job : job - R;
        const int64_t r = ray0 + slot;
        if (r >= B) continue;
        float* base = tail_lds + (size_t)slot * per_ray;
        if (job < R) {
            if constexpr (TRAIN) {
                composite_train_wave<true>(raw, z, rays, noise, noise_std, white_back, a->target, a->grad_scale, nullptr, rgb, depth, opac,
                                           fine_pass ? a->g_raw_fine : a->g_raw_coarse, r, S, base, nullptr, lane);
            } else if (TT && !fine_pass) {
                composite_fwd_wave<1>(raw, z, rays, noise, noise_std, white_back, nullptr, nullptr, nullptr, opac, r, S, nullptr, lane);
            } else {
                composite_fwd_wave<4>(raw, z, rays, noise, noise_std, white_back, nullptr, rgb, depth, opac, r, S, nullptr, lane);
            }
        } else {
            float* w_s = base + S4;
            composite_weights_wave<(TT ? 1 : 4)>(raw, z, rays, noise, noise_std, r, S, w_s, lane);
            __builtin_amdgcn_wave_barrier();
            const float* u = a->u;
            fine_z_wave(w_s + S4, z + r * S, [&](int j) { return w_s[1 + j]; }, u ? u + r * a->u_stride : nullptr, S, N_i, a->eps,
                        a->z_fine + r * S_f, nullptr, nullptr, nullptr, lane, a->row_total);
        }
    }
}

template <int PREC, int SV>
__global__ __launch_bounds__(PrecTraits<PREC>::NW * 64, PrecTraits<PREC>::WPS)
void mlp_render_kernel(const RenderArgs args_by_value) {
    constexpr bool TRAIN = SV == 1 || SV == 2, TT = SV == 3;
    constexpr int FSV = TT ? 0 : SV;
    constexpr int NW = PrecTraits<PREC>::NW, PTS = 32 * NW, R = kRenderRays;
    __shared__ __attribute__((aligned(1024))) char lds_all[FwdLds<PREC, TRAIN>::kBytes];
    __shared__ float red[2][16];
    __shared__ unsigned last_s;
    const int lane = threadIdx.x & 63;
    const int wave = __builtin_amdgcn_readfirstlane((int)(threadIdx.x >> 6));
    float* const tail_lds = reinterpret_cast<float*>(lds_all + FwdLds<PREC, TRAIN>::kRingOff);
    int nc, nf;
    {
        const RenderArgsP a = render_args();
        const int S_c = a->S_c, N_i = a->N_i;
        nc = R * S_c / PTS;
        nf = N_i > 0 ? R * (S_c + N_i) / PTS : 0;
    }
    const int total = nc + nf;
#pragma clang loop unroll(disable)
    for (int sp = 0; sp < total; ++sp) {
        if (sp > 0) render_wg_sync();
        if (sp == nc) {
            render_tail<TRAIN, NW, TT>(false, true, tail_lds, wave, lane);
            render_wg_sync();
        }
        const RenderArgsP a = render_args();
        const bool fine = sp >= nc;
        const int S = fine ? a->S_c + a->N_i : a->S_c;
        const unsigned blk = fine ? blockIdx.x * (unsigned)nf + (unsigned)(sp - nc) : blockIdx.x * (unsigned)nc + (unsigned)sp;
        const FwdZGen zg{fine ? nullptr : a->perturb_rand, fine ? nullptr : a->z_coarse, fine ? 0 : a->use_disp, fine ? 0.0f : a->perturb,
                          TRAIN ? a->regen_enc : 0};
        uint8_t* save = nullptr;
        if constexpr (TRAIN) save = (uint8_t*)(fine ? a->save_fine : a->save_coarse);
        if (TT && !fine)
            mlp_fwd_body<PREC, MODE_RAYS, true, 0>(lds_all, blk, a->rays, nullptr, a->B * (int64_t)S, (int64_t)S, (const uint8_t*)a->packed_coarse,
                                                   a->raw_coarse, nullptr, zg);
        else
            mlp_fwd_body<PREC, MODE_RAYS, false, FSV>(lds_all, blk, a->rays, fine ? a->z_fine : nullptr, a->B * (int64_t)S, (int64_t)S,
                                                      (const uint8_t*)(fine ? a->packed_fine : a->packed_coarse), fine ? a->raw_fine : a->raw_coarse, save, zg);
    }
    render_wg_sync();
    render_tail<TRAIN, NW, TT>(nf > 0, false, tail_lds, wave, lane);

    if constexpr (TRAIN) {
        const RenderArgsP a = render_args();
        unsigned* const ticket = a->ticket;
        asm volatile("s_waitcnt vmcnt(0)" ::: "memory");
        __syncthreads();
        if (threadIdx.x == 0) {
            const unsigned prev = __hip_atomic_fetch_add(ticket, 1u, __ATOMIC_RELAXED, __HIP_MEMORY_SCOPE_AGENT);
            last_s = (prev == gridDim.x - 1) ? 1u : 0u;
            if (prev == gridDim.x - 1) __hip_atomic_store(ticket, 0u, __ATOMIC_RELAXED, __HIP_MEMORY_SCOPE_AGENT);
        }
        __syncthreads();
        if (!last_s) return;
        __builtin_amdgcn_fence(__ATOMIC_ACQUIRE, "agent");
        const float* img_c = a->rgb_coarse;
        const float* img_f = a->rgb_fine;
        const float* target = a->target;
        float* out3 = a->out3;
        const int64_t n3 = 3 * a->B;
        auto fresh_c = [&](int64_t i) { return __hip_atomic_load(img_c + i, __ATOMIC_RELAXED, __HIP_MEMORY_SCOPE_AGENT); };
        auto fresh_f = [&](int64_t i) { return __hip_atomic_load(img_f + i, __ATOMIC_RELAXED, __HIP_MEMORY_SCOPE_AGENT); };
        constexpr int Q = 1024 / (NW * 64);
        if (nf > 0)
            mse_psnr_block<Q>(fresh_c, fresh_f, true, target, n3, out3, nullptr, nullptr, red);
        else
            mse_psnr_block<Q>(fresh_c, [&](int64_t i) { return 0.0f; }, false, target, n3, out3, nullptr, nullptr, red);
    }
}

template <int PREC, int SV>
int launch_render_variant(const RenderArgs& a, unsigned groups, hipStream_t stream);

}
```

nerf_pl_amd/models/train_step.py:

```python
import os

import numpy as np
import torch

from .. import ops


def fusable(models, embeddings, loss_mod):
    from ..losses import MSELoss
    from .rendering import _fusable
    return (isinstance(loss_mod, MSELoss) and _fusable(models, embeddings)
            and len({m.mlp_dtype for m in models}) == 1
            and all(p.requires_grad for m in models for p in m.parameters()))


def _forward_launches(models, rays, rgbs, S, N, dtype, use_disp, perturb, perturb_rand, noise_c, noise_f, noise_std, white_back, u, gscale,
                      packs, acts_c, dev):
    z, raw_c = ops.mlp_fwd_rays_coarse(rays, S, packs[0][0], False, dtype, use_disp, perturb, perturb_rand, save=acts_c)
    if N > 0:
        _, opac_c, rgb_c, depth_c, g_raw_c, zf = ops.composite_train_fine_z(raw_c, z, rays, noise_c, noise_std, white_back, rgbs,
                                                                            gscale, N, u=u)
        acts_f = ops.alloc_acts(zf.numel(), dtype, dev)
        raw_f = ops.mlp_fwd_rays(rays, zf, packs[1][0], False, dtype, save=acts_f)
        opac_f, rgb_f, depth_f, g_raw_f, out3 = ops.composite_train_loss(raw_f, zf, rays, noise_f, noise_std, white_back, rgbs,
                                                                        gscale, rgb_coarse=rgb_c)
        entries = [(g_raw_f, raw_f, packs[1][1], acts_f), (g_raw_c, raw_c, packs[0][1], acts_c)]
        outs = [rgb_c, depth_c, opac_c, rgb_f, depth_f, opac_f]
    else:
        opac_c, rgb_c, depth_c, g_raw_c, out3 = ops.composite_train_loss(raw_c, z, rays, noise_c, noise_std, white_back, rgbs, gscale)
        entries = [(g_raw_c, raw_c, packs[0][1], acts_c)]
        outs = [rgb_c, depth_c, opac_c]
    return outs, entries, out3


def _tracked(model):
    ref = getattr(model, "_serial_tracked", None)
    return ref is not None and ref() is not None


_regen_enc = os.environ.get("NERFHIP_REGEN_ENC", "0") == "1"


def regen_enc_enabled():
    return _regen_enc


def set_regen_enc(on):
    global _regen_enc
    prev, _regen_enc = _regen_enc, bool(on)
    return prev


class _TrainRender(torch.autograd.Function):
    @staticmethod
    def forward(ctx, cfg, rays, rgbs, *params):
        models, S, use_disp, perturb, noise_std, N, white_back, adam, draws, packed = cfg
        rays = rays.float().contiguous()
        rgbs = rgbs.float().contiguous()
        B = rays.shape[0]
        dev = rays.device
        dtype = models[0].mlp_dtype
        if draws is None:
            from .. import draws as D
            draws = D.step_draws(B, S, N, perturb, noise_std, dev)
        perturb_rand = draws.get("perturb_rand") if perturb > 0 else None
        noise_c, noise_f = draws.get("noise_coarse"), draws.get("noise_fine")
        u = draws.get("u") if (N > 0 and perturb != 0) else None
        if noise_std != 0 and (noise_c is None or (N > 0 and noise_f is None)):
            raise ValueError("render_rays_train: noise_std != 0 needs the noise draws")
        fresh = (packed is not None and packed[0] == tuple(id(m) for m in models) and packed[1] == dtype
                 and all(_tracked(m) and getattr(m, "_weights_serial", 0) == sr
                         and getattr(m, "_packed_serial", None) == sr for m, sr in zip(models, packed[2])))
        packs = [m.train_buffers(dtype, dev) for m in models] if fresh else ops.pack_models_train(models, dtype)
        gscale = float(np.float32(2.0) / np.float32(3 * B))
        acts_c = ops.alloc_acts(B * S, dtype, dev)
        if ops.render_supported(B, S, N, dtype):
            acts_f = ops.alloc_acts(B * (S + N), dtype, dev) if N > 0 else None
            regen = regen_enc_enabled() and ops.mlp_dtype_code(dtype) == ops.BF16 and S % 32 == 0 and (S + N) % 32 == 0
            o = ops.render_train_fwd(rays, rgbs, gscale, S, N, packs[0][0], packs[1][0] if N > 0 else None, dtype, acts_c, acts_f,
                                     use_disp, perturb, perturb_rand, noise_c, noise_f, noise_std, white_back, u, regen_enc=regen)
            out3 = o["out3"]
            outs = [o["rgb_coarse"], o["depth_coarse"], o["opacity_coarse"]]
            entries = [(o["g_raw_coarse"], o["raw_coarse"], packs[0][1], acts_c) + ((rays, o["z_coarse"]) if regen else ())]
            if N > 0:
                outs += [o["rgb_fine"], o["depth_fine"], o["opacity_fine"]]
                entries.insert(0, (o["g_raw_fine"], o["raw_fine"], packs[1][1], acts_f) + ((rays, o["z_fine"]) if regen else ()))
        else:
            outs, entries, out3 = _forward_launches(models, rays, rgbs, S, N, dtype, use_disp, perturb, perturb_rand, noise_c, noise_f, noise_std,
                                                    white_back, u, gscale, packs, acts_c, dev)
        ctx.models = [models[1], models[0]] if N > 0 else [models[0]]
        ctx.entries, ctx.dtype, ctx.adam = entries, dtype, adam
        ctx.n_params = [len(m.flat_params()) for m in models]
        ctx.serials = [m._packed_serial for m in ctx.models]
        ctx.mark_non_differentiable(out3, *outs)
        ctx.set_materialize_grads(False)
        return (out3[0], out3) + tuple(outs)

    @staticmethod
    def backward(ctx, g_loss, *_unused):
        n_models = len(ctx.n_params)
        if g_loss is None:
            return (None, None, None) + (None,) * sum(ctx.n_params)
        entries = ctx.entries
        g_scale = None if ops.is_unit_seed(g_loss) else g_loss.reshape(1).float().contiguous()
        models, dtype = ctx.models, ctx.dtype
        for m, serial in zip(models, ctx.serials):
            m.check_pack_serial(serial)
        hooked = any(getattr(m, "_grad_ready_hook", None) is not None for m in models)
        joint_hook = getattr(models[0], "_grads_ready_hook", None) if hooked else None
        if hooked and joint_hook is not None and all(getattr(m, "_grads_ready_hook", None) == joint_hook for m in models):
            grads = ops.mlp_bwd_multi(entries, dtype, g_scale=g_scale)
            for m, g in zip(models, grads):
                m._flat_grad = g[2]
            joint_hook(models, [g[2] for g in grads])
        elif hooked:
            grads = []
            for m, entry in zip(models, entries):
                ((gw, gb, flat),) = ops.mlp_bwd_multi([entry], dtype, g_scale=g_scale)
                m._flat_grad = flat
                m._grad_ready_hook(m, flat)
                grads.append((gw, gb, flat))
        else:
            if ctx.adam is not None and any(p.grad is not None for m in models for p in m.flat_params()):
                ctx.adam = None
            adam = ctx.adam.handle(models) if ctx.adam is not None else None
            grads = ops.mlp_bwd_multi(entries, dtype, adam=adam, g_scale=g_scale)
            for m, g in zip(models, grads):
                m._flat_grad = g[2]
            if ctx.adam is not None:
                ctx.adam.applied_in_backward(models)
        ctx.entries = None
        by_model = {id(m): g for m, g in zip(models, grads)}
        out = []
        order = [models[-1]] + models[:-1] if n_models == 2 else models
        for m in order:
            gw, gb, _ = by_model[id(m)]
            out += gw + gb
        return (None, None, None) + tuple(out)


def render_rays_train(models, embeddings, rays, rgbs, N_samples=64, use_disp=False, perturb=0, noise_std=1, N_importance=0,
                      white_back=False, adam=None, draws=None, packed=None):
    N = int(N_importance)
    use = list(models[:2]) if N > 0 else [models[0]]
    params = [p for m in use for p in m.flat_params()]
    cfg = (use, int(N_samples), bool(use_disp), float(perturb), float(noise_std), N, bool(white_back), adam, draws, packed)
    res = _TrainRender.apply(cfg, rays, rgbs, *params)
    loss, out3 = res[0], res[1]
    results = {'rgb_coarse': res[2], 'depth_coarse': res[3], 'opacity_coarse': res[4]}
    if N > 0:
        results.update(rgb_fine=res[5], depth_fine=res[6], opacity_fine=res[7])
    return results, loss, out3
```

nerf_pl_amd/ops.py:

```python
import ctypes
import os

import torch

from . import _lib
from ._lib import BF16, BF16_F8, F32, NerfHipError, check, device_guard, ptr, require_gpu, stream_ptr

_DTYPES = {"fp32": F32, "f32": F32, "float32": F32, torch.float32: F32, F32: F32,
           "bf16": BF16, "bfloat16": BF16, torch.bfloat16: BF16, "bf16_f8": BF16_F8}


def mlp_dtype_code(d):
    if isinstance(d, bool) or d not in _DTYPES:
        raise ValueError("mlp dtype must be 'fp32', 'bf16' or 'bf16_f8', got %r" % (d,))
    return _DTYPES[d]


def _c(t):
    return t if t.is_contiguous() else t.contiguous()


def _check_draw(op, name, t, numel):
    if t is not None and (t.numel() != numel or t.dtype != torch.float32):
        raise ValueError("%s: %s must hold %d fp32 draws, got %s %s" % (op, name, numel, tuple(t.shape), t.dtype))


def _noise_arg(op, name, noise, noise_std, numel):
    if noise_std == 0 or noise is None:
        return None
    noise = _c(noise)
    _check_draw(op, name, noise, numel)
    return noise


def _u_arg(op, u, B, K):
    if u is None:
        return None, 0
    if tuple(u.shape) not in ((B, K), (K,)) or u.dtype != torch.float32:
        raise ValueError("%s: u must be (N_importance,) or (B, N_importance) = (%d, %d) fp32, got %s %s"
                         % (op, B, K, tuple(u.shape), u.dtype))
    return _c(u), (K if u.dim() == 2 else 0)


def _perturb_arg(op, perturb, perturb_rand, numel):
    if not perturb > 0:
        return None
    if perturb_rand is None:
        raise ValueError("%s: perturb>0 needs perturb_rand" % op)
    perturb_rand = _c(perturb_rand)
    _check_draw(op, "perturb_rand", perturb_rand, numel)
    return perturb_rand


def _train_composite_args(op, raw, z, rays, target):
    raw, z, rays, target = _c(raw), _c(z), _c(rays), _c(target)
    B, S = z.shape
    if raw.numel() != B * S * 4 or target.numel() != B * 3:
        raise ValueError("%s: raw must be (B,S,4) and target (B,3)" % op)
    return raw, z, rays, target, B, S


def _train_composite_outs(B, S, dev):
    f32 = dict(device=dev, dtype=torch.float32)
    return torch.empty(B, **f32), torch.empty(B, 3, **f32), torch.empty(B, **f32), torch.empty(B, S, 4, **f32)


_TICKETS = {}
_CAPTURES = {}
_EAGER_SLOTS = {}
_TICKET_WORDS = 1024


def _ticket(device):
    st = torch.cuda.current_stream(device)
    capturing = torch.cuda.is_current_stream_capturing()
    rec = _CAPTURES.setdefault((device.index, st.stream_id), [False, 0])
    if capturing and not rec[0]:
        rec[1] += 1
    rec[0] = capturing
    pool = _TICKETS.get(device.index)
    if pool is None:
        if capturing:
            raise NerfHipError("the ticket words of this GPU must exist before a capture: run the step once eagerly first")
        pool = _TICKETS[device.index] = torch.zeros(_TICKET_WORDS * 4, device=device, dtype=torch.int32)
    if capturing:
        slot = 32 + rec[1] % (_TICKET_WORDS - 32)
    else:
        slot = _EAGER_SLOTS.setdefault((device.index, st.stream_id), len([k for k in _EAGER_SLOTS if k[0] == device.index]) % 32)
    return pool[4 * slot:4 * slot + 4]


class _PosEnc(torch.autograd.Function):
    @staticmethod
    def forward(ctx, x, n_freqs, bands):
        require_gpu(x, bands)
        x = _c(x)
        n, C = x.shape
        out = torch.empty(n, C * (2 * n_freqs + 1), device=x.device, dtype=torch.float32)
        check(_lib.load().nerfhip_posenc_bands(ptr(x), ptr(bands), ptr(out), n, C, n_freqs, stream_ptr()), "nerfhip_posenc")
        ctx.save_for_backward(x)
        ctx.n_freqs, ctx.bands = n_freqs, bands
        return out

    @staticmethod
    def backward(ctx, gout):
        (x,) = ctx.saved_tensors
        gout = _c(gout.float())
        gx = torch.empty_like(x)
        n, C = x.shape
        check(_lib.load().nerfhip_posenc_bands_bwd(ptr(x), ptr(ctx.bands), ptr(gout), ptr(gx), n, C, ctx.n_freqs, stream_ptr()),
              "nerfhip_posenc_bwd")
        return gx, None, None


@device_guard
def posenc(x, n_freqs, bands=None):
    if x.dim() != 2:
        raise ValueError("posenc expects (n, C)")
    if bands is not None:
        if bands.numel() != int(n_freqs):
            raise ValueError("posenc: need one band per frequency")
        bands = bands.to(x.device, torch.float32).contiguous()
    return _PosEnc.apply(x, int(n_freqs), bands)


@device_guard
def sample_coarse_z(rays, n_samples, use_disp=False, perturb=0.0, perturb_rand=None):
    require_gpu(rays, perturb_rand)
    rays = _c(rays)
    B = rays.shape[0]
    perturb_rand = _perturb_arg("sample_coarse_z", perturb, perturb_rand, B * n_samples)
    z = torch.empty(B, n_samples, device=rays.device, dtype=torch.float32)
    check(_lib.load().nerfhip_sample_coarse_z(ptr(rays), ptr(perturb_rand), ptr(z), B, n_samples, int(bool(use_disp)),
                                              float(perturb), stream_ptr()), "nerfhip_sample_coarse_z")
    return z


@device_guard
def searchsorted(a, v, out=None, side="left"):
    require_gpu(a, v)
    if side not in ("left", "right"):
        raise ValueError("side must be 'left' or 'right'")
    if a.dim() != 2 or v.dim() != 2 or not (a.shape[0] == v.shape[0] or a.shape[0] == 1 or v.shape[0] == 1):
        raise ValueError("searchsorted expects a (B,M) and v (B,K), or one of them with a single row")
    rows = max(a.shape[0], v.shape[0])
    a, v = _c(a.expand(rows, a.shape[1])), _c(v.expand(rows, v.shape[1]))
    B, M = a.shape
    K = v.shape[1]
    if out is None:
        out = torch.empty(B, K, device=a.device, dtype=torch.int64)
    elif out.dtype != torch.int64 or not out.is_contiguous() or tuple(out.shape) != (B, K):
        raise ValueError("out must be a contiguous int64 (B,K) tensor")
    fn = _lib.load().nerfhip_searchsorted_right if side == "right" else _lib.load().nerfhip_searchsorted_left
    check(fn(ptr(a), ptr(v), ptr(out), B, M, K, stream_ptr()), "nerfhip_searchsorted_" + side)
    return out


_ROW_TOTAL_MODES = {"exact": 0, "aten": 1}
_row_total = _ROW_TOTAL_MODES[os.environ.get("NERFHIP_ROW_TOTAL", "aten")]


def set_row_total(mode):
    global _row_total
    prev = [k for k, v in _ROW_TOTAL_MODES.items() if v == _row_total][0]
    _row_total = _ROW_TOTAL_MODES[mode]
    return prev


@device_guard
def sample_pdf_u(bins, weights, n_importance, u=None, eps=1e-5, return_cdf_inds=False):
    require_gpu(bins, weights, u)
    if bins.stride(-1) != 1:
        bins = bins.contiguous()
    if weights.stride(-1) != 1:
        weights = weights.contiguous()
    B, M = weights.shape
    if bins.shape != (B, M + 1):
        raise ValueError("bins must be (N_rays, N_samples_+1)")
    u, u_stride = _u_arg("sample_pdf", u, B, n_importance)
    samples = torch.empty(B, n_importance, device=bins.device, dtype=torch.float32)
    cdf = torch.empty(B, M + 1, device=bins.device, dtype=torch.float32) if return_cdf_inds else None
    inds = torch.empty(B, n_importance, device=bins.device, dtype=torch.int64) if return_cdf_inds else None
    check(_lib.load().nerfhip_sample_pdf_ex(ptr(bins), bins.stride(0), ptr(weights), weights.stride(0), ptr(u), u_stride,
                                            ptr(samples), B, M, n_importance, float(eps), ptr(cdf), ptr(inds), _row_total,
                                            stream_ptr()),
          "nerfhip_sample_pdf")
    return (samples, cdf, inds) if return_cdf_inds else samples


@device_guard
def fine_z(z_coarse, w_coarse, n_importance, u=None, eps=1e-5, return_new=False, return_cdf_inds=False):
    require_gpu(z_coarse, w_coarse, u)
    z_coarse, w_coarse = _c(z_coarse), _c(w_coarse)
    B, S = z_coarse.shape
    u, u_stride = _u_arg("fine_z", u, B, n_importance)
    zf = torch.empty(B, S + n_importance, device=z_coarse.device, dtype=torch.float32)
    zn = torch.empty(B, n_importance, device=z_coarse.device, dtype=torch.float32) if return_new else None
    cdf = torch.empty(B, S - 1, device=z_coarse.device, dtype=torch.float32) if return_cdf_inds else None
    inds = torch.empty(B, n_importance, device=z_coarse.device, dtype=torch.int64) if return_cdf_inds else None
    check(_lib.load().nerfhip_fine_z_ex(ptr(z_coarse), ptr(w_coarse), ptr(u), u_stride, ptr(zf), ptr(zn), B, S,
                                        n_importance, float(eps), ptr(cdf), ptr(inds), _row_total, stream_ptr()), "nerfhip_fine_z")
    out = (zf, zn) if return_new else (zf,)
    if return_cdf_inds:
        out = out + (cdf, inds)
    return out if len(out) > 1 else out[0]


class _Composite(torch.autograd.Function):
    @staticmethod
    def forward(ctx, raw, z, rays, noise, noise_std, white_back):
        require_gpu(raw, z, rays, noise)
        raw, z, rays = _c(raw), _c(z), _c(rays)
        B, S = z.shape
        raw_ch = 4 if raw.dim() == 3 else 1
        if raw.numel() != B * S * raw_ch:
            raise ValueError("raw must be (B,S,4) or (B,S)")
        if noise is not None:
            noise = _c(noise)
        dev = z.device
        weights = torch.empty(B, S, device=dev, dtype=torch.float32)
        opacity = torch.empty(B, device=dev, dtype=torch.float32)
        rgb = torch.empty(B, 3, device=dev, dtype=torch.float32) if raw_ch == 4 else None
        depth = torch.empty(B, device=dev, dtype=torch.float32) if raw_ch == 4 else None
        check(_lib.load().nerfhip_composite_fwd(ptr(raw), raw_ch, ptr(z), ptr(rays), ptr(noise), float(noise_std),
                                                int(bool(white_back)), ptr(weights), ptr(rgb), ptr(depth),
                                                ptr(opacity), B, S, stream_ptr()), "nerfhip_composite_fwd")
        ctx.save_for_backward(raw, z, rays, noise)
        ctx.cfg = (raw_ch, float(noise_std), int(bool(white_back)))
        ctx.set_materialize_grads(False)
        if raw_ch == 4:
            return weights, opacity, rgb, depth
        return weights, opacity

    @staticmethod
    def backward(ctx, g_weights, g_opacity, g_rgb=None, g_depth=None):
        raw, z, rays, noise = ctx.saved_tensors
        raw_ch, noise_std, white_back = ctx.cfg
        B, S = z.shape

        def prep(g):
            return None if g is None else _c(g.float())

        g_raw = torch.empty_like(raw)
        check(_lib.load().nerfhip_composite_bwd(ptr(raw), raw_ch, ptr(z), ptr(rays), ptr(noise), noise_std, white_back,
                                                ptr(prep(g_rgb)), ptr(prep(g_depth)), ptr(prep(g_opacity)),
                                                ptr(prep(g_weights)), ptr(g_raw), B, S, stream_ptr()),
              "nerfhip_composite_bwd")
        return g_raw, None, None, None, None, None


@device_guard
def composite(raw, z, rays, noise=None, noise_std=0.0, white_back=False):
    if noise_std == 0:
        noise = None
    return _Composite.apply(raw, z, rays, noise, float(noise_std), bool(white_back))


@device_guard
def composite_train(raw, z, rays, noise, noise_std, white_back, target, grad_scale, want_weights=True):
    require_gpu(raw, z, rays, noise, target)
    raw, z, rays, target, B, S = _train_composite_args("composite_train", raw, z, rays, target)
    noise = _noise_arg("composite_train", "noise", noise, noise_std, B * S)
    weights = torch.empty(B, S, device=z.device, dtype=torch.float32) if want_weights else None
    opacity, rgb, depth, g_raw = _train_composite_outs(B, S, z.device)
    check(_lib.load().nerfhip_composite_train(ptr(raw), ptr(z), ptr(rays), ptr(noise), float(noise_std), int(bool(white_back)),
                                              ptr(target), float(grad_scale), ptr(weights), ptr(rgb), ptr(depth), ptr(opacity),
                                              ptr(g_raw), B, S, stream_ptr()), "nerfhip_composite_train")
    return weights, opacity, rgb, depth, g_raw


@device_guard
def composite_train_fine_z(raw, z, rays, noise, noise_std, white_back, target, grad_scale, n_importance, u=None, eps=1e-5,
                           want_weights=False):
    require_gpu(raw, z, rays, noise, target, u)
    raw, z, rays, target, B, S = _train_composite_args("composite_train_fine_z", raw, z, rays, target)
    noise = _noise_arg("composite_train_fine_z", "noise", noise, noise_std, B * S)
    u, u_stride = _u_arg("composite_train_fine_z", u, B, n_importance)
    dev = z.device
    weights = torch.empty(B, S, device=dev, dtype=torch.float32) if want_weights else None
    opacity, rgb, depth, g_raw = _train_composite_outs(B, S, dev)
    zf = torch.empty(B, S + n_importance, device=dev, dtype=torch.float32)
    check(_lib.load().nerfhip_composite_train_fine_z(ptr(raw), ptr(z), ptr(rays), ptr(noise), float(noise_std), int(bool(white_back)),
                                                     ptr(target), float(grad_scale), ptr(weights), ptr(rgb), ptr(depth), ptr(opacity),
                                                     ptr(g_raw), B, S, ptr(u), u_stride, int(n_importance), float(eps), ptr(zf),
                                                     _row_total, stream_ptr()), "nerfhip_composite_train_fine_z")
    return weights, opacity, rgb, depth, g_raw, zf


@device_guard
def composite_train_loss(raw, z, rays, noise, noise_std, white_back, target, grad_scale, rgb_coarse=None):
    require_gpu(raw, z, rays, noise, target, rgb_coarse)
    raw, z, rays, target, B, S = _train_composite_args("composite_train_loss", raw, z, rays, target)
    if rgb_coarse is not None:
        rgb_coarse = _c(rgb_coarse)
        if rgb_coarse.numel() != B * 3:
            raise ValueError("composite_train_loss: rgb_coarse must be (B,3)")
    noise = _noise_arg("composite_train_loss", "noise", noise, noise_std, B * S)
    dev = z.device
    opacity, rgb, depth, g_raw = _train_composite_outs(B, S, dev)
    out3 = torch.empty(3, device=dev, dtype=torch.float32)
    check(_lib.load().nerfhip_composite_train_loss(ptr(raw), ptr(z), ptr(rays), ptr(noise), float(noise_std), int(bool(white_back)),
                                                   ptr(target), float(grad_scale), None, ptr(rgb), ptr(depth), ptr(opacity), ptr(g_raw),
                                                   B, S, ptr(rgb_coarse), ptr(out3), ptr(_ticket(dev)), stream_ptr()),
          "nerfhip_composite_train_loss")
    return opacity, rgb, depth, g_raw, out3


class _MsePsnr(torch.autograd.Function):
    @staticmethod
    def forward(ctx, rgb_c, rgb_f, target):
        require_gpu(rgb_c, rgb_f, target)
        rgb_c, target = _c(rgb_c), _c(target)
        rgb_f = _c(rgb_f) if rgb_f is not None else None
        n = target.numel()
        if rgb_c.numel() != n or (rgb_f is not None and rgb_f.numel() != n):
            raise ValueError("mse_psnr: shape mismatch")
        out3 = torch.empty(3, device=target.device, dtype=torch.float32)
        g_c = torch.empty_like(rgb_c)
        g_f = torch.empty_like(rgb_f) if rgb_f is not None else None
        check(_lib.load().nerfhip_mse_psnr(ptr(rgb_c), ptr(rgb_f), ptr(target), n, ptr(out3), ptr(g_c), ptr(g_f), stream_ptr()),
              "nerfhip_mse_psnr")
        ctx.save_for_backward(g_c, g_f)
        ctx.mark_non_differentiable(out3)
        ctx.set_materialize_grads(False)
        return out3[0], out3

    @staticmethod
    def backward(ctx, g_loss, _g_out3):
        g_c, g_f = ctx.saved_tensors
        if g_loss is None:
            return None, None, None
        if is_unit_seed(g_loss):
            return g_c, g_f, None
        if g_f is None:
            return g_c * g_loss, None, None
        g_c, g_f = torch._foreach_mul([g_c, g_f], g_loss)
        return g_c, g_f, None


_UNIT_SEEDS = {}


def unit_seed(like):
    key = (like.device.type, like.device.index)
    t = _UNIT_SEEDS.get(key)
    if t is None:
        t = _UNIT_SEEDS[key] = torch.ones((), device=like.device, dtype=torch.float32)
    return t


def is_unit_seed(g):
    t = _UNIT_SEEDS.get((g.device.type, g.device.index))
    return t is not None and g.data_ptr() == t.data_ptr() and g.numel() == 1


@device_guard
def mse_psnr_values(rgb_coarse, rgb_fine, target):
    require_gpu(rgb_coarse, rgb_fine, target)
    rgb_coarse, target = _c(rgb_coarse), _c(target)
    rgb_fine = _c(rgb_fine) if rgb_fine is not None else None
    out3 = torch.empty(3, device=target.device, dtype=torch.float32)
    check(_lib.load().nerfhip_mse_psnr(ptr(rgb_coarse), ptr(rgb_fine), ptr(target), target.numel(), ptr(out3), None, None, stream_ptr()),
          "nerfhip_mse_psnr")
    return out3


@device_guard
def mse_psnr(rgb_coarse, rgb_fine, target):
    return _MsePsnr.apply(rgb_coarse, rgb_fine, target)


PARAM_ORDER = ["xyz_encoding_1.0", "xyz_encoding_2.0", "xyz_encoding_3.0", "xyz_encoding_4.0",
               "xyz_encoding_5.0", "xyz_encoding_6.0", "xyz_encoding_7.0", "xyz_encoding_8.0",
               "xyz_encoding_final", "dir_encoding.0", "sigma", "rgb.0"]
PARAM_SHAPES = [(256, 63), (256, 256), (256, 256), (256, 256), (256, 319), (256, 256), (256, 256), (256, 256),
                (256, 256), (128, 283), (1, 256), (3, 128)]


DEFAULT_ARCH_ONLY = "the fused HIP MLP implements the reference's default architecture (D=8, W=256, skips=[4], 63/27 inputs) only"


def packed_bytes(dtype):
    return int(_lib.load().nerfhip_mlp_packed_bytes(mlp_dtype_code(dtype)))


def packed_bwd_bytes(dtype):
    return int(_lib.load().nerfhip_mlp_packed_bwd_bytes(mlp_dtype_code(dtype)))


def pack_arg_tables(weights, biases):
    if len(weights) != 12 or len(biases) != 12:
        raise ValueError("need 12 weights and 12 biases")
    for i, (w, b) in enumerate(zip(weights, biases)):
        require_gpu(w, b)
        if tuple(w.shape) != PARAM_SHAPES[i] or tuple(b.shape) != (PARAM_SHAPES[i][0],):
            raise NerfHipError("%s; got %s for %s" % (DEFAULT_ARCH_ONLY, tuple(w.shape), PARAM_ORDER[i]))
        if not (w.is_contiguous() and b.is_contiguous()):
            raise NerfHipError("NeRF parameters must be contiguous")
    wp = (ctypes.c_void_p * 12)(*[w.data_ptr() for w in weights])
    bp = (ctypes.c_void_p * 12)(*[b.data_ptr() for b in biases])
    return wp, bp


@device_guard
def pack_weights_raw(wp, bp, out, dtype):
    check(_lib.load().nerfhip_mlp_pack_weights(wp, bp, ptr(out), mlp_dtype_code(dtype), stream_ptr()), "nerfhip_mlp_pack_weights")


@device_guard
def pack_weights_bwd_raw(wp, bp, out, dtype):
    check(_lib.load().nerfhip_mlp_pack_weights_bwd(wp, bp, ptr(out), mlp_dtype_code(dtype), stream_ptr()),
          "nerfhip_mlp_pack_weights_bwd")


@device_guard
def pack_weights_train_raw(wp, bp, out, out_bwd, dtype):
    check(_lib.load().nerfhip_mlp_pack_weights_train(wp, bp, ptr(out), ptr(out_bwd), mlp_dtype_code(dtype), stream_ptr()),
          "nerfhip_mlp_pack_weights_train")


def alloc_acts(n_points, dtype, device):
    nbytes = int(_lib.load().nerfhip_mlp_act_bytes(int(n_points), mlp_dtype_code(dtype)))
    return torch.empty(nbytes, device=device, dtype=torch.uint8)


@device_guard
def mlp_fwd_embedded(x, packed, sigma_only, dtype, save=None):
    require_gpu(x)
    if x.dim() != 2 or x.stride(1) != 1:
        x = x.reshape(-1, x.shape[-1]).contiguous()
    n = x.shape[0]
    need = 63 if sigma_only else 90
    if x.shape[1] != need:
        raise ValueError("NeRF.forward expects %d input channels, got %d" % (need, x.shape[1]))
    out = torch.empty(n, 1 if sigma_only else 4, device=x.device, dtype=torch.float32)
    check(_lib.load().nerfhip_mlp_fwd_embedded(ptr(x), x.stride(0), n, ptr(packed), ptr(out), int(bool(sigma_only)),
                                               mlp_dtype_code(dtype), ptr(save), stream_ptr()),
          "nerfhip_mlp_fwd_embedded")
    return out


@device_guard
def mlp_fwd_rays(rays, z, packed, sigma_only, dtype, save=None):
    require_gpu(rays, z)
    rays, z = _c(rays), _c(z)
    B, S = z.shape
    out = torch.empty((B, S) if sigma_only else (B, S, 4), device=z.device, dtype=torch.float32)
    check(_lib.load().nerfhip_mlp_fwd_rays(ptr(rays), ptr(z), B, S, ptr(packed), ptr(out), int(bool(sigma_only)),
                                           mlp_dtype_code(dtype), ptr(save), stream_ptr()), "nerfhip_mlp_fwd_rays")
    return out


@device_guard
def mlp_fwd_rays_coarse(rays, n_samples, packed, sigma_only, dtype, use_disp=False, perturb=0.0, perturb_rand=None, save=None):
    require_gpu(rays, perturb_rand)
    rays = _c(rays)
    B, S = rays.shape[0], int(n_samples)
    perturb_rand = _perturb_arg("mlp_fwd_rays_coarse", perturb, perturb_rand, B * S)
    z = torch.empty(B, S, device=rays.device, dtype=torch.float32)
    out = torch.empty((B, S) if sigma_only else (B, S, 4), device=rays.device, dtype=torch.float32)
    check(_lib.load().nerfhip_mlp_fwd_rays_coarse(ptr(rays), ptr(perturb_rand), ptr(z), B, S,
                                                  int(bool(use_disp)), float(perturb), ptr(packed), ptr(out), int(bool(sigma_only)),
                                                  mlp_dtype_code(dtype), ptr(save), stream_ptr()), "nerfhip_mlp_fwd_rays_coarse")
    return z, out


_render_fused = os.environ.get("NERFHIP_RENDER_FUSED", "1") != "0"


def set_render_fused(on):
    global _render_fused
    prev, _render_fused = _render_fused, bool(on)
    return prev


def render_supported(B, S_c, N_i, dtype):
    if not _render_fused:
        return False
    return bool(_lib.load().nerfhip_render_supported(int(B), int(S_c), int(N_i), mlp_dtype_code(dtype)))


def _render_args(rays, S, N, packed_c, packed_f, use_disp, perturb, perturb_rand, noise_c, noise_f, noise_std, white_back, u, eps,
                 want_coarse, coarse_sigma_only=False):
    B = rays.shape[0]
    dev = rays.device
    f32 = dict(device=dev, dtype=torch.float32)
    a = _lib.RenderArgs()
    bufs = {"z_coarse": torch.empty(B, S, **f32), "opacity_coarse": torch.empty(B, **f32),
            "raw_coarse": torch.empty((B, S) if coarse_sigma_only else (B, S, 4), **f32)}
    if want_coarse:
        bufs.update(rgb_coarse=torch.empty(B, 3, **f32), depth_coarse=torch.empty(B, **f32))
    if N > 0:
        bufs.update(z_fine=torch.empty(B, S + N, **f32), raw_fine=torch.empty(B, S + N, 4, **f32), rgb_fine=torch.empty(B, 3, **f32),
                    depth_fine=torch.empty(B, **f32), opacity_fine=torch.empty(B, **f32))
    perturb_rand = _perturb_arg("render", perturb, perturb_rand, B * S)
    noise_c = _noise_arg("render", "noise_coarse", noise_c, noise_std, B * S)
    noise_f = _noise_arg("render", "noise_fine", noise_f if N > 0 else None, noise_std, B * (S + N))
    if noise_std != 0 and (noise_c is None or (N > 0 and noise_f is None)):
        raise ValueError("render: noise_std != 0 needs the noise draws")
    u, u_stride = _u_arg("render", u if N > 0 else None, B, N)
    a.rays, a.B, a.S_c, a.N_i = rays.data_ptr(), B, int(S), int(N)
    a.packed_coarse = packed_c.data_ptr()
    a.packed_fine = packed_f.data_ptr() if packed_f is not None else None
    for k, t in bufs.items():
        setattr(a, k, t.data_ptr())
    a.perturb_rand = perturb_rand.data_ptr() if perturb_rand is not None else None
    a.perturb, a.use_disp = float(perturb), int(bool(use_disp))
    a.noise_coarse = noise_c.data_ptr() if noise_c is not None else None
    a.noise_fine = noise_f.data_ptr() if noise_f is not None else None
    a.noise_std, a.white_back = float(noise_std), int(bool(white_back))
    a.u, a.u_stride, a.eps, a.row_total = (u.data_ptr() if u is not None else None), u_stride, float(eps), _row_total
    keep = (rays, packed_c, packed_f, perturb_rand, noise_c, noise_f, u)
    return a, bufs, keep


@device_guard
def render_fwd(rays, n_samples, n_importance, packed_coarse, packed_fine, dtype, use_disp=False, perturb=0.0, perturb_rand=None,
               noise_coarse=None, noise_fine=None, noise_std=0.0, white_back=False, u=None, eps=1e-5, want_coarse=True, test_time=False):
    require_gpu(rays, perturb_rand, noise_coarse, noise_fine, u)
    rays = _c(rays)
    tt = bool(test_time) and int(n_importance) > 0
    a, bufs, keep = _render_args(rays, n_samples, n_importance, packed_coarse, packed_fine, use_disp, perturb, perturb_rand,
                                 noise_coarse, noise_fine, noise_std, white_back, u, eps, want_coarse and not tt, coarse_sigma_only=tt)
    if tt:
        check(_lib.load().nerfhip_render_test_fwd(ctypes.addressof(a), mlp_dtype_code(dtype), stream_ptr()), "nerfhip_render_test_fwd")
    else:
        check(_lib.load().nerfhip_render_fwd(ctypes.addressof(a), mlp_dtype_code(dtype), stream_ptr()), "nerfhip_render_fwd")
    return bufs


@device_guard
def render_train_fwd(rays, target, grad_scale, n_samples, n_importance, packed_coarse, packed_fine, dtype, acts_coarse, acts_fine,
                     use_disp=False, perturb=0.0, perturb_rand=None, noise_coarse=None, noise_fine=None, noise_std=0.0,
                     white_back=False, u=None, eps=1e-5, regen_enc=False):
    require_gpu(rays, target, perturb_rand, noise_coarse, noise_fine, u)
    rays, target = _c(rays), _c(target)
    B, S, N = rays.shape[0], int(n_samples), int(n_importance)
    if target.numel() != 3 * B or target.dtype != torch.float32:
        raise ValueError("render_train_fwd: target must be (B,3) fp32")
    a, bufs, keep = _render_args(rays, S, N, packed_coarse, packed_fine, use_disp, perturb, perturb_rand, noise_coarse, noise_fine,
                                 noise_std, white_back, u, eps, True)
    dev = rays.device
    bufs["g_raw_coarse"] = torch.empty(B, S, 4, device=dev, dtype=torch.float32)
    if N > 0:
        bufs["g_raw_fine"] = torch.empty(B, S + N, 4, device=dev, dtype=torch.float32)
    bufs["out3"] = torch.empty(3, device=dev, dtype=torch.float32)
    a.g_raw_coarse = bufs["g_raw_coarse"].data_ptr()
    a.g_raw_fine = bufs["g_raw_fine"].data_ptr() if N > 0 else None
    a.out3 = bufs["out3"].data_ptr()
    a.save_coarse = acts_coarse.data_ptr()
    a.save_fine = acts_fine.data_ptr() if N > 0 else None
    a.target, a.grad_scale = target.data_ptr(), float(grad_scale)
    a.ticket = _ticket(dev).data_ptr()
    a.regen_enc = int(bool(regen_enc) and mlp_dtype_code(dtype) == BF16)
    check(_lib.load().nerfhip_render_train_fwd(ctypes.addressof(a), mlp_dtype_code(dtype), stream_ptr()), "nerfhip_render_train_fwd")
    return bufs


FLAT_GRAD_FLOATS = sum(s[0] * s[1] + s[0] for s in PARAM_SHAPES)


def flat_grad_views(n_points, device, shapes=PARAM_SHAPES, out=None):
    sizes = [s[0] * s[1] for s in shapes] + [s[0] for s in shapes]
    if out is not None:
        flat = out
        if n_points == 0:
            flat.zero_()
    else:
        flat = (torch.zeros if n_points == 0 else torch.empty)(sum(sizes), device=device, dtype=torch.float32)
    views, off = [], 0
    for sz in sizes:
        views.append(flat[off:off + sz])
        off += sz
    return [v.view(s) for v, s in zip(views[:12], shapes)], views[12:], flat


@device_guard
def mlp_bwd(g_out, out, packed_bwd, acts, dtype, shapes=PARAM_SHAPES, phases=7, workspace=None):
    require_gpu(g_out, out)
    code = mlp_dtype_code(dtype)
    g_out = _c(g_out.float()).reshape(-1, 4)
    out = _c(out).reshape(-1, 4)
    n = out.shape[0]
    dev = out.device
    lib = _lib.load()
    if workspace is not None and "dys" in workspace:
        dys, ws = workspace["dys"], workspace["ws"]
    else:
        dys = torch.empty(int(lib.nerfhip_mlp_dy_bytes(n, code)), device=dev, dtype=torch.uint8)
        ws = torch.empty(int(lib.nerfhip_mlp_dw_workspace_bytes(n, code)), device=dev, dtype=torch.uint8)
        if workspace is not None:
            workspace["dys"], workspace["ws"] = dys, ws
    gw, gb, flat = flat_grad_views(n, dev, shapes)
    gwp = (ctypes.c_void_p * 12)(*[t.data_ptr() for t in gw])
    gbp = (ctypes.c_void_p * 12)(*[t.data_ptr() for t in gb])
    check(lib.nerfhip_mlp_bwd_phases(ptr(g_out), ptr(out), n, ptr(packed_bwd), ptr(acts), ptr(dys), ptr(ws), gwp, gbp, 0, code,
                                     int(phases), stream_ptr()), "nerfhip_mlp_bwd")
    return gw, gb, flat


@device_guard
def mlp_dx_embedded(dys, n, w_xyz1, w_xyz5, w_dir, dtype):
    code = mlp_dtype_code(dtype)
    if code == BF16_F8:
        raise NotImplementedError("nerfhip_mlp_dx_embedded reads bf16 / fp32 dY slabs ('bf16_f8' keeps dY only as e5m2: NeRF.forward "
                                  "saves in bf16 for calls whose input requires grad, models/mlp_autograd.py)")
    require_gpu(w_xyz1, w_xyz5, w_dir)
    gx = torch.empty(n, 90, device=dys.device, dtype=torch.float32)
    check(_lib.load().nerfhip_mlp_dx_embedded(ptr(dys), n, ptr(_c(w_xyz1.detach())), ptr(_c(w_xyz5.detach())), ptr(_c(w_dir.detach())),
                                              ptr(gx), 90, code, stream_ptr()), "nerfhip_mlp_dx_embedded")
    return gx


def pack_tables(models, dtype):
    if not 1 <= len(models) <= 4:
        raise ValueError("pack_models_train packs 1..4 models")
    tabs, bufs = [], []
    for m in models:
        if not m.is_default_arch():
            raise NotImplementedError(DEFAULT_ARCH_ONLY)
        wp, bp, dev = m._pack_args()
        tabs.append((wp, bp))
        bufs.append(m.train_buffers(dtype, dev))
    n = len(models)
    W = (ctypes.c_void_p * (12 * n))(*[t[0][i] for t in tabs for i in range(12)])
    Bv = (ctypes.c_void_p * (12 * n))(*[t[1][i] for t in tabs for i in range(12)])
    P = (ctypes.c_void_p * n)(*[b[0].data_ptr() for b in bufs])
    Pb = (ctypes.c_void_p * n)(*[b[1].data_ptr() for b in bufs])
    return W, Bv, P, Pb, bufs


def mark_packed(models):
    for m in models:
        m._packed_serial = getattr(m, "_weights_serial", 0)


def pack_models_train(models, dtype):
    W, Bv, P, Pb, bufs = pack_tables(models, dtype)
    with torch.cuda.device(bufs[0][0].device):
        check(_lib.load().nerfhip_mlp_pack_weights_train_multi(W, Bv, P, Pb, len(models), mlp_dtype_code(dtype), stream_ptr()),
              "nerfhip_mlp_pack_weights_train_multi")
    mark_packed(models)
    return bufs


def mlp_bwd_multi(entries, dtype, adam=None, phases=7, workspace=None, g_scale=None):
    code = mlp_dtype_code(dtype)
    lib = _lib.load()
    M = len(entries)
    dev = entries[0][1].device
    gs, outs, ns, dys, grads = [], [], [], [], []
    enc, keep_enc = None, []
    for m, e in enumerate(entries):
        g_out, out = e[0], e[1]
        if len(e) > 4 and e[4] is not None:
            if enc is None:
                enc = _lib.EncSource()
            rays_e, z_e = _c(e[4]), _c(e[5])
            require_gpu(rays_e, z_e)
            if rays_e.dtype != torch.float32 or z_e.dtype != torch.float32 or z_e.dim() != 2 or rays_e.shape[0] != z_e.shape[0]:
                raise ValueError("mlp_bwd_multi: (rays (B,8), z (B,S)) fp32 expected")
            enc.rays[m], enc.z[m], enc.S[m] = rays_e.data_ptr(), z_e.data_ptr(), int(z_e.shape[1])
            keep_enc.append((rays_e, z_e))
        require_gpu(g_out, out)
        g_out = _c(g_out.float()).reshape(-1, 4)
        out = _c(out).reshape(-1, 4)
        gs.append(g_out)
        outs.append(out)
        ns.append(out.shape[0])
    with torch.cuda.device(dev):
        n_arr = (ctypes.c_int64 * M)(*ns)
        key = ("multi", tuple(ns), code)
        if workspace is not None and key in workspace:
            dys, ws = workspace[key]
        else:
            dys = [torch.empty(int(lib.nerfhip_mlp_dy_bytes(n, code)), device=dev, dtype=torch.uint8) for n in ns]
            ws = torch.empty(int(lib.nerfhip_mlp_dw_workspace_bytes_multi(n_arr, M, code)), device=dev, dtype=torch.uint8)
            if workspace is not None:
                workspace[key] = (dys, ws)
        joint = torch.empty(M * FLAT_GRAD_FLOATS, device=dev, dtype=torch.float32)
        for m, n in enumerate(ns):
            grads.append(flat_grad_views(n, dev, out=joint[m * FLAT_GRAD_FLOATS:(m + 1) * FLAT_GRAD_FLOATS]))
        vp = ctypes.c_void_p
        G = (vp * M)(*[t.data_ptr() for t in gs])
        O = (vp * M)(*[t.data_ptr() for t in outs])
        PB = (vp * M)(*[e[2].data_ptr() for e in entries])
        AC = (vp * M)(*[e[3].data_ptr() for e in entries])
        DY = (vp * M)(*[t.data_ptr() for t in dys])
        GW = (vp * (12 * M))(*[t.data_ptr() for g in grads for t in g[0]])
        GB = (vp * (12 * M))(*[t.data_ptr() for g in grads for t in g[1]])
        if adam is not None:
            for m in range(M):
                adam.grad_flat[m] = grads[m][2].data_ptr()
        if g_scale is not None:
            require_gpu(g_scale)
        check(lib.nerfhip_mlp_bwd_multi_rays(M, G, O, n_arr, PB, AC, DY, ptr(ws), GW, GB, 0, code, int(phases), ptr(g_scale),
                                             ctypes.addressof(adam) if adam is not None else None,
                                             ctypes.addressof(enc) if enc is not None else None, stream_ptr()), "nerfhip_mlp_bwd_multi_rays")
    return grads


ACT_NONE, ACT_RELU, ACT_SIGMOID = 0, 1, 2


def _rows(t):
    if t.dim() != 2:
        raise ValueError("expected a (n, channels) tensor")
    if t.stride(1) != 1 or t.stride(0) < t.shape[1]:
        t = t.contiguous()
    return t


def _off(t, col):
    return ctypes.c_void_p(t.data_ptr() + 4 * col)


class _LinearAct(torch.autograd.Function):

    @staticmethod
    def forward(ctx, act, dtype, w, b, *xs):
        xs = [_rows(x.float()) for x in xs]
        require_gpu(w, b, *xs)
        w, b = _c(w), _c(b)
        n, n_out, k_tot = xs[0].shape[0], w.shape[0], w.shape[1]
        if sum(x.shape[1] for x in xs) != k_tot or any(x.shape[0] != n for x in xs) or b.numel() != n_out:
            raise ValueError("linear: input segments %s do not match the weight %s" % ([tuple(x.shape) for x in xs], tuple(w.shape)))
        lib = _lib.load()
        code = mlp_dtype_code(dtype)
        y = torch.empty(n, n_out, device=w.device, dtype=torch.float32)
        col = 0
        for s, x in enumerate(xs):
            last = s == len(xs) - 1
            check(lib.nerfhip_linear_fwd(ptr(x), x.stride(0), _off(w, col), k_tot, ptr(b) if last else None, ptr(y), n_out, n,
                                         x.shape[1], n_out, act if last else ACT_NONE, int(s > 0), code, stream_ptr()),
                  "nerfhip_linear_fwd")
            col += x.shape[1]
        ctx.cfg = (act, code)
        ctx.save_for_backward(w, y, *xs)
        return y

    @staticmethod
    def backward(ctx, gy):
        w, y, *xs = ctx.saved_tensors
        act, code = ctx.cfg
        lib = _lib.load()
        gy = _c(gy.float())
        n, n_out, k_tot = y.shape[0], w.shape[0], w.shape[1]
        need_w, need_b = ctx.needs_input_grad[2], ctx.needs_input_grad[3]
        gw = gb = None
        gxs = []
        if (need_w or need_b) and n > 0:
            gw = torch.empty_like(w)
            gb = torch.empty(n_out, device=w.device, dtype=torch.float32)
            ws_bytes = max(lib.nerfhip_linear_bwd_weight_workspace_bytes(n, x.shape[1], n_out) for x in xs)
            ws = torch.empty(ws_bytes, device=w.device, dtype=torch.uint8)
        elif need_w or need_b:
            gw, gb = torch.zeros_like(w), torch.zeros(n_out, device=w.device, dtype=torch.float32)
        col = 0
        for s, x in enumerate(xs):
            if (need_w or need_b) and n > 0:
                check(lib.nerfhip_linear_bwd_weight(ptr(gy), n_out, ptr(y), n_out, act, ptr(x), x.stride(0), _off(gw, col), k_tot,
                                                    ptr(gb) if s == 0 else None, ptr(ws), n, x.shape[1], n_out, 0, code,
                                                    stream_ptr()), "nerfhip_linear_bwd_weight")
            gx = None
            if ctx.needs_input_grad[4 + s]:
                gx = torch.empty(n, x.shape[1], device=w.device, dtype=torch.float32)
                check(lib.nerfhip_linear_bwd_input(ptr(gy), n_out, ptr(y), n_out, act, _off(w, col), k_tot, ptr(gx), x.shape[1], n,
                                                   x.shape[1], n_out, 0, code, stream_ptr()), "nerfhip_linear_bwd_input")
            gxs.append(gx)
            col += x.shape[1]
        return (None, None, gw if need_w else None, gb if need_b else None) + tuple(gxs)


@device_guard
def linear_act(xs, weight, bias, act, dtype):
    return _LinearAct.apply(int(act), dtype, weight, bias, *xs)


_INT32_MAX = 2 ** 31 - 1


def _require_mesh(name, t, dtype, shape_len=None, cols=None):
    if not torch.is_tensor(t):
        raise NerfHipError("%s: expected a torch tensor, got %s" % (name, type(t).__name__))
    if not t.is_cuda:
        raise NerfHipError("nerf_pl_amd runs on MI355X only: %s is a %s tensor (no CPU fallback)" % (name, t.device))
    if t.dtype != dtype:
        raise NerfHipError("%s: expected %s, got %s" % (name, dtype, t.dtype))
    if shape_len is not None and t.dim() != shape_len:
        raise NerfHipError("%s: expected rank %d, got shape %s" % (name, shape_len, tuple(t.shape)))
    if cols is not None and t.shape[-1] != cols:
        raise NerfHipError("%s: expected %d columns, got shape %s" % (name, cols, tuple(t.shape)))
    return _c(t)


def _check_vertex_ids(triangles, V):
    if triangles.numel() and (int(triangles.min()) < 0 or int(triangles.max()) >= V):
        raise NerfHipError("triangles reference vertices outside [0, %d)" % V)


@device_guard
def marching_cubes(volume, iso):
    volume = _require_mesh("marching_cubes volume", volume, torch.float32, 3)
    n0, n1, n2 = volume.shape
    if min(n0, n1, n2) < 2:
        raise NerfHipError("marching_cubes: every dimension must be >= 2, got %s" % (tuple(volume.shape),))
    lib = _lib.load()
    ws_bytes = lib.nerfhip_marching_cubes_workspace_bytes(n0, n1, n2)
    if ws_bytes == 0:
        raise NerfHipError("marching_cubes: volume %s has 2^31 or more lattice points" % (tuple(volume.shape),))
    ws = torch.empty(ws_bytes, device=volume.device, dtype=torch.uint8)
    totals = torch.empty(2, device=volume.device, dtype=torch.int64)
    check(lib.nerfhip_marching_cubes_count(ptr(volume), n0, n1, n2, float(iso), ptr(ws), ptr(totals), stream_ptr()),
          "nerfhip_marching_cubes_count")
    V, T = (int(x) for x in totals.cpu())
    if V > _INT32_MAX or T > _INT32_MAX:
        raise NerfHipError("marching_cubes: %d vertices / %d triangles do not fit int32" % (V, T))
    verts = torch.empty(V, 3, device=volume.device, dtype=torch.float64)
    tris = torch.empty(T, 3, device=volume.device, dtype=torch.int32)
    if V or T:
        check(lib.nerfhip_marching_cubes_emit(ptr(volume), n0, n1, n2, float(iso), ptr(ws), ptr(totals), ptr(verts), ptr(tris),
                                              stream_ptr()), "nerfhip_marching_cubes_emit")
    return verts, tris


@device_guard
def largest_cluster(triangles, n_vertices):
    triangles = _require_mesh("triangles", triangles, torch.int32, 2, 3)
    T, V = triangles.shape[0], int(n_vertices)
    dev = triangles.device
    if T == 0 or V == 0:
        return torch.empty(0, device=dev, dtype=torch.int64), torch.empty(0, 3, device=dev, dtype=torch.int32)
    if V > _INT32_MAX or 3 * T > _INT32_MAX:
        raise NerfHipError("largest_cluster: mesh too large (V=%d, T=%d)" % (V, T))
    _check_vertex_ids(triangles, V)
    lib = _lib.load()
    keys = torch.empty(3 * T, device=dev, dtype=torch.int64)
    check(lib.nerfhip_mesh_edge_keys(ptr(triangles), T, ptr(keys), stream_ptr()), "nerfhip_mesh_edge_keys")
    sorted_keys, order = torch.sort(keys, stable=True)
    ws = torch.empty(lib.nerfhip_mesh_cluster_workspace_bytes(V, T), device=dev, dtype=torch.uint8)
    totals = torch.empty(3, device=dev, dtype=torch.int64)
    check(lib.nerfhip_mesh_largest_cluster(ptr(triangles), V, T, ptr(sorted_keys), ptr(order), ptr(ws), ptr(totals), stream_ptr()),
          "nerfhip_mesh_largest_cluster")
    t_kept, v_kept, status = (int(x) for x in totals.cpu())
    if status:
        raise NerfHipError("largest_cluster: the union-find gave up after its retry bound")
    kept_ids = torch.empty(v_kept, device=dev, dtype=torch.int64)
    kept_tris = torch.empty(t_kept, 3, device=dev, dtype=torch.int32)
    check(lib.nerfhip_mesh_cluster_compact(ptr(triangles), V, T, ptr(ws), ptr(kept_ids), ptr(kept_tris), stream_ptr()),
          "nerfhip_mesh_cluster_compact")
    return kept_ids, kept_tris


@device_guard
def vertex_normals(vertices, triangles):
    vertices = _require_mesh("vertices", vertices, torch.float32, 2, 3)
    triangles = _require_mesh("triangles", triangles, torch.int32, 2, 3)
    V, T = vertices.shape[0], triangles.shape[0]
    out = torch.empty(V, 3, device=vertices.device, dtype=torch.float64)
    if V == 0:
        return out
    _check_vertex_ids(triangles, V)
    check(_lib.load().nerfhip_mesh_vertex_normals(ptr(vertices), V, ptr(triangles), T, ptr(out), stream_ptr()),
          "nerfhip_mesh_vertex_normals")
    return out


@device_guard
def normal_rays(vertices, normals, near, far, near_t):
    vertices = _require_mesh("vertices", vertices, torch.float32, 2, 3)
    normals = _require_mesh("normals", normals, torch.float64, 2, 3)
    V = vertices.shape[0]
    rays = torch.empty(V, 8, device=vertices.device, dtype=torch.float32)
    if V:
        check(_lib.load().nerfhip_mesh_normal_rays(ptr(vertices), ptr(normals), V, float(near), float(far), float(near_t), ptr(rays),
                                                   stream_ptr()), "nerfhip_mesh_normal_rays")
    return rays


@device_guard
def view_rays(vertices, w2c, origin, focal, image, near):
    import numpy as np
    vertices = _require_mesh("vertices", vertices, torch.float32, 2, 3)
    image = _require_mesh("image", image, torch.uint8, 3, 3)
    H, W = image.shape[0], image.shape[1]
    V = vertices.shape[0]
    dev = vertices.device
    colors = torch.empty(V, 4, device=dev, dtype=torch.uint8)
    depth = torch.empty(V, device=dev, dtype=torch.float64)
    rays = torch.empty(V, 8, device=dev, dtype=torch.float32)
    if V:
        w = np.ascontiguousarray(np.asarray(w2c, np.float32).reshape(3, 4))
        o = np.ascontiguousarray(np.asarray(origin, np.float32).reshape(3))
        fp = ctypes.POINTER(ctypes.c_float)
        check(_lib.load().nerfhip_mesh_view_rays(ptr(vertices), V, w.ctypes.data_as(fp), o.ctypes.data_as(fp), float(np.float32(focal)),
                                                 W, H, ptr(image), float(near), ptr(colors), ptr(depth), ptr(rays), stream_ptr()),
              "nerfhip_mesh_view_rays")
    return colors, depth, rays


@device_guard
def color_accumulate(colors, depth, opacity, occ_threshold, accum):
    colors = _require_mesh("colors", colors, torch.uint8, 2, 4)
    depth = _require_mesh("depth", depth, torch.float64, 1)
    opacity = _require_mesh("opacity", opacity, torch.float32, 1)
    accum = _require_mesh("accum", accum, torch.float64, 2, 4)
    V = colors.shape[0]
    if V:
        check(_lib.load().nerfhip_mesh_color_accumulate(ptr(colors), ptr(depth), ptr(opacity), V, float(occ_threshold), ptr(accum),
                                                        stream_ptr()), "nerfhip_mesh_color_accumulate")
    return accum


@device_guard
def color_finish(accum):
    accum = _require_mesh("accum", accum, torch.float64, 2, 4)
    V = accum.shape[0]
    out = torch.empty(V, 3, device=accum.device, dtype=torch.uint8)
    if V:
        check(_lib.load().nerfhip_mesh_color_finish(ptr(accum), V, ptr(out), stream_ptr()), "nerfhip_mesh_color_finish")
    return out


@device_guard
def rgb_to_u8(rgb):
    rgb = _require_mesh("rgb", rgb, torch.float32)
    out = torch.empty(rgb.shape, device=rgb.device, dtype=torch.uint8)
    if rgb.numel():
        check(_lib.load().nerfhip_mesh_rgb_to_u8(ptr(rgb), rgb.numel(), ptr(out), stream_ptr()), "nerfhip_mesh_rgb_to_u8")
    return out


IMAGE_PLANAR, IMAGE_INTERLEAVED = 0, 1


@device_guard
def ssim(img1, img2, B, C, H, W, window_size=3, layout=IMAGE_PLANAR, want_map=False, want_mean=True):
    require_gpu(img1, img2)
    B, C, H, W, window_size = int(B), int(C), int(H), int(W), int(window_size)
    if min(B, C, H, W) < 0 or img1.numel() != B * C * H * W or img2.numel() != img1.numel():
        raise NerfHipError("ssim: images of %s and %s elements are not %d x %d x %d x %d" % (img1.numel(), img2.numel(), B, C, H, W))
    if window_size % 2 == 0 or not 3 <= window_size <= 11:
        raise NerfHipError("ssim: window_size must be odd and in 3..11, got %d" % window_size)
    img1, img2 = _c(img1), _c(img2)
    dev = img1.device
    lib = _lib.load()
    shape = (B, C, H, W) if layout == IMAGE_PLANAR else (B, H, W, C)
    out_map = torch.empty(shape, device=dev, dtype=torch.float32) if want_map else None
    mean = ws = None
    if want_mean:
        mean = torch.full((), float("nan"), device=dev, dtype=torch.float32) if img1.numel() == 0 else \
            torch.empty((), device=dev, dtype=torch.float32)
        ws = torch.empty(max(1, lib.nerfhip_ssim_workspace_bytes(B, C, H, W) // 8), device=dev, dtype=torch.float64)
    check(lib.nerfhip_ssim(ptr(img1), ptr(img2), B, C, H, W, window_size, int(layout), ptr(out_map), ptr(mean), ptr(ws), stream_ptr()),
          "nerfhip_ssim")
    return out_map, mean


def _require_depth_table(table, device):
    if not torch.is_tensor(table) or not table.is_cuda or table.dtype != torch.uint8 or tuple(table.shape) != (256, 3) \
            or table.device != device:
        raise NerfHipError("depth_colormap: the colour table must be a (256, 3) uint8 tensor on %s" % (device,))
    return _c(table)


@device_guard
def depth_colormap(depth, table, want_float=True, want_bytes=False):
    require_gpu(depth)
    table = _require_depth_table(table, depth.device)
    depth = _c(depth)
    n, dev = depth.numel(), depth.device
    lib = _lib.load()
    out_f = torch.empty((3,) + tuple(depth.shape), device=dev, dtype=torch.float32) if want_float else None
    out_b = torch.empty(tuple(depth.shape) + (3,), device=dev, dtype=torch.uint8) if want_bytes else None
    ws = torch.empty(max(1, lib.nerfhip_depth_colormap_workspace_bytes(n) // 4), device=dev, dtype=torch.float32)
    check(lib.nerfhip_depth_colormap(ptr(depth), n, ptr(table), ptr(out_f), ptr(out_b), ptr(ws), stream_ptr()),
          "nerfhip_depth_colormap")
    return out_f, out_b


GIF_STRIP = 3838


def gif_workspace(F, H, W, device):
    nbytes = _lib.load().nerfhip_gif_workspace_bytes(F, H, W)
    if F > 0 and nbytes == 0:
        raise NerfHipError("gif: %d frames of %d x %d are refused (1..65535 per side, at most 2^26 pixels, at most 65535 frames)"
                           % (F, H, W))
    return torch.empty(max(1, nbytes // 8), device=device, dtype=torch.int64)


@device_guard
def gif_quantize(frames, workspace=None):
    frames = _require_u8("gif_quantize: frames", frames)
    if frames.dim() != 4 or frames.shape[3] != 3:
        raise NerfHipError("gif_quantize: expected (F, H, W, 3), got %s" % (tuple(frames.shape),))
    F, H, W = frames.shape[:3]
    dev = frames.device
    lib = _lib.load()
    ws = workspace if workspace is not None else gif_workspace(F, H, W, dev)
    indices = torch.empty((F, H * W), device=dev, dtype=torch.uint8)
    palettes = torch.empty((F, 256, 3), device=dev, dtype=torch.uint8)
    boxes = torch.empty((F,), device=dev, dtype=torch.int32)
    check(lib.nerfhip_gif_quantize(ptr(frames), F, H, W, ptr(indices), ptr(palettes), ptr(boxes), ptr(ws), stream_ptr()),
          "nerfhip_gif_quantize")
    return indices, palettes, boxes


@device_guard
def gif_lzw(indices, H, W, workspace=None):
    indices = _require_u8("gif_lzw: indices", indices)
    if indices.dim() != 2 or indices.shape[1] != H * W:
        raise NerfHipError("gif_lzw: expected (F, %d) indices for %d x %d frames, got %s" % (H * W, H, W, tuple(indices.shape)))
    F = indices.shape[0]
    dev = indices.device
    lib = _lib.load()
    ws = workspace if workspace is not None else gif_workspace(F, H, W, dev)
    stride = lib.nerfhip_gif_data_stride(H, W)
    data = torch.empty((F, stride), device=dev, dtype=torch.uint8)
    lengths = torch.empty((F,), device=dev, dtype=torch.int32)
    check(lib.nerfhip_gif_lzw(ptr(indices), F, H, W, ptr(data), ptr(lengths), ptr(ws), stream_ptr()), "nerfhip_gif_lzw")
    return data, lengths


def _require_u8(name, t):
    if not torch.is_tensor(t):
        raise NerfHipError("%s: expected a torch tensor, got %s" % (name, type(t).__name__))
    if not t.is_cuda:
        raise NerfHipError("nerf_pl_amd runs on MI355X only: %s is a %s tensor (no CPU fallback)" % (name, t.device))
    if t.dtype != torch.uint8:
        raise NerfHipError("%s: expected uint8, got %s" % (name, t.dtype))
    return _c(t)


@device_guard
def decode_png_batch(streams, H, W, ch, return_flags=False):
    streams = _require_u8("decode_png_batch streams", streams)
    H, W, ch = int(H), int(W), int(ch)
    if ch not in (1, 3, 4) or H < 1 or W < 1:
        raise NerfHipError("decode_png_batch: H, W >= 1 and ch in (1, 3, 4), got %d x %d x %d" % (H, W, ch))
    if streams.dim() != 2 or streams.shape[1] != H * (1 + W * ch):
        raise NerfHipError("decode_png_batch: expected (n, %d) bytes per %d x %d x %d image, got %s"
                           % (H * (1 + W * ch), H, W, ch, tuple(streams.shape)))
    n = streams.shape[0]
    out = torch.empty(n, H, W, ch, device=streams.device, dtype=torch.uint8)
    flags = torch.empty(n, device=streams.device, dtype=torch.int32)
    check(_lib.load().nerfhip_png_unfilter(ptr(streams), ptr(out), ptr(flags), n, H, W, ch, stream_ptr()), "nerfhip_png_unfilter")
    if return_flags:
        return out, flags
    if n and bool(flags.any()):
        raise NerfHipError("decode_png_batch: image(s) %s hold a scanline filter type above 4" % flags.nonzero().flatten().tolist())
    return out


_TAPS = {}


def _lanczos_taps_device(in_size, out_size, device):
    key = (int(in_size), int(out_size), str(device))
    if key not in _TAPS:
        from .imageio_min import lanczos_taps
        if len(_TAPS) > 16:
            _TAPS.clear()
        _TAPS[key] = tuple(torch.from_numpy(a).to(device) for a in lanczos_taps(in_size, out_size))
    return _TAPS[key]


@device_guard
def resize_rgba_lanczos(u8, w, h):
    u8 = _require_u8("resize_rgba_lanczos image", u8)
    if u8.dim() not in (3, 4) or u8.shape[-1] != 4:
        raise NerfHipError("resize_rgba_lanczos: expected (n, H, W, 4) or (H, W, 4), got %s" % (tuple(u8.shape),))
    w, h = int(w), int(h)
    single = u8.dim() == 3
    n, H, W = (1,) + tuple(u8.shape[:2]) if single else tuple(u8.shape[:3])
    if min(w, h, H, W) < 1:
        raise NerfHipError("resize_rgba_lanczos: empty image")
    dev = u8.device
    out = torch.empty(n, h, w, 4, device=dev, dtype=torch.uint8)
    th = _lanczos_taps_device(W, w, dev) if W != w else (None, None, None)
    tv = _lanczos_taps_device(H, h, dev) if H != h else (None, None, None)
    ws = torch.empty(n, H, w, 4, device=dev, dtype=torch.uint8) if (W != w and H != h) else None
    check(_lib.load().nerfhip_resize_rgba_lanczos(ptr(u8), ptr(out), ptr(ws), n, H, W, h, w, ptr(th[0]), ptr(th[1]), ptr(th[2]),
                                                  th[2].shape[1] if th[2] is not None else 0, ptr(tv[0]), ptr(tv[1]), ptr(tv[2]),
                                                  tv[2].shape[1] if tv[2] is not None else 0, stream_ptr()),
          "nerfhip_resize_rgba_lanczos")
    return out[0] if single else out


@device_guard
def rgba_to_rgb_white(u8, out=None):
    u8 = _require_u8("rgba_to_rgb_white image", u8)
    if u8.dim() < 1 or u8.shape[-1] != 4:
        raise NerfHipError("rgba_to_rgb_white: expected (..., 4) uint8, got %s" % (tuple(u8.shape),))
    n = u8.numel() // 4
    if out is None:
        out = torch.empty(n, 3, device=u8.device, dtype=torch.float32)
    else:
        require_gpu(out)
        if out.device != u8.device or tuple(out.shape) != (n, 3) or not out.is_contiguous():
            raise NerfHipError("rgba_to_rgb_white: out must be a contiguous (%d, 3) float32 tensor on %s" % (n, u8.device))
    mask = torch.empty(n, device=u8.device, dtype=torch.uint8)
    check(_lib.load().nerfhip_rgba_to_rgb_white(ptr(u8), ptr(out), ptr(mask), n, stream_ptr()), "nerfhip_rgba_to_rgb_white")
    return out, mask.view(torch.bool)


def jpeg_entropy_decode(parsed):
    import numpy as np
    comps = parsed["components"]
    mx, my = int(parsed["mcus_x"]), int(parsed["mcus_y"])
    table = np.zeros((8, 272), np.uint8)
    mask = 0
    for (tc, th), (counts, symbols) in parsed["huffman"].items():
        table[4 * tc + th, :16] = counts
        table[4 * tc + th, 16:16 + len(symbols)] = symbols
        mask |= 1 << (4 * tc + th)
    comp = np.ascontiguousarray([[c[1], c[2], c[4], c[5]] for c in comps], dtype=np.int32)
    coef = [np.zeros((my * c[2], mx * c[1], 64), np.int16) for c in comps]
    scan = np.frombuffer(parsed["scan"], np.uint8)
    ptrs = (ctypes.c_void_p * len(comps))(*[a.ctypes.data for a in coef])
    caps = (ctypes.c_int64 * len(comps))(*[a.shape[0] * a.shape[1] for a in coef])
    code = _lib.load().nerfhip_jpeg_entropy_decode(scan.ctypes.data, len(scan), len(comps), comp.ctypes.data, table.ctypes.data, mask,
                                                   mx, my, int(parsed["restart_interval"]), ptrs, caps)
    if code != 0:
        msg = _lib.load().nerfhip_error_string(code).decode()
        raise NerfHipError("%s: nerfhip_jpeg_entropy_decode failed: %s (code %d)" % (parsed.get("name", "JPEG data"), msg, code))
    return coef


def _require_i16(name, t, device, shape):
    if not torch.is_tensor(t):
        raise NerfHipError("%s: expected a torch tensor, got %s" % (name, type(t).__name__))
    if not t.is_cuda:
        raise NerfHipError("nerf_pl_amd runs on MI355X only: %s is a %s tensor (no CPU fallback)" % (name, t.device))
    if t.dtype != torch.int16 or tuple(t.shape) != tuple(shape) or (device is not None and t.device != device):
        raise NerfHipError("%s: expected int16 %s on %s, got %s %s on %s" % (name, tuple(shape), device, t.dtype, tuple(t.shape), t.device))
    return _c(t)


@device_guard
def decode_jpeg_batch(coefs, quant, H, W, hs=1, vs=1):
    if torch.is_tensor(coefs):
        coefs = [coefs]
    coefs = list(coefs)
    H, W, hs, vs = int(H), int(W), int(hs), int(vs)
    n_comp = len(coefs)
    lib = _lib.load()
    plane_bytes = lib.nerfhip_jpeg_planes_bytes(H, W, n_comp, hs, vs) if n_comp in (1, 3) else 0
    if plane_bytes == 0:
        raise NerfHipError("decode_jpeg_batch: %d component(s) of %d x %d with luma sampling %dx%d is not supported (1 component, "
                           "or 3 with 1x1, 2x1 or 2x2)" % (n_comp, W, H, hs, vs))
    if not torch.is_tensor(coefs[0]) or coefs[0].dim() < 2:
        raise NerfHipError("decode_jpeg_batch: coefs must be (n, blocks, 64) int16 tensors")
    n, dev = coefs[0].shape[0], coefs[0].device
    mx, my = -(-W // (8 * hs)), -(-H // (8 * vs))
    flat = []
    for c, t in enumerate(coefs):
        blocks = mx * my * (hs * vs if c == 0 else 1)
        if torch.is_tensor(t) and t.dim() == 4:
            t = t.reshape(t.shape[0], -1, 64)
        flat.append(_require_i16("decode_jpeg_batch coefs[%d]" % c, t, dev, (n, blocks, 64)))
    quant = _require_i16("decode_jpeg_batch quant", quant, dev, (n, n_comp, 64))
    out = torch.empty(n, H, W, 4, device=dev, dtype=torch.uint8)
    planes = torch.empty(n * plane_bytes, device=dev, dtype=torch.uint8)
    check(lib.nerfhip_jpeg_decode(ptr(flat[0]), ptr(flat[1]) if n_comp == 3 else None, ptr(flat[2]) if n_comp == 3 else None,
                                  ptr(quant), ptr(planes), ptr(out), n, H, W, n_comp, hs, vs, stream_ptr()), "nerfhip_jpeg_decode")
    return out
```

nerf_pl_amd/system.py:

```python
import os
from collections import defaultdict

import torch
from torch import nn

from .losses import loss_dict
from .metrics import psnr
from .models.nerf import Embedding, NeRF
from .models.rendering import render_rays

try:
    from pytorch_lightning import LightningModule as _Base
except Exception:
    _Base = nn.Module


def get_learning_rate(optimizer):
    for g in optimizer.param_groups:
        return g['lr']


class NeRFSystem(_Base):
    def __init__(self, hparams, train_dataset=None, val_dataset=None):
        super(NeRFSystem, self).__init__()
        self.hparams_ = hparams
        try:
            self.hparams = hparams
        except Exception:
            pass
        self.loss = loss_dict[getattr(hparams, 'loss_type', 'mse')]()
        self.embedding_xyz = Embedding(3, 10)
        self.embedding_dir = Embedding(3, 4)
        self.embeddings = [self.embedding_xyz, self.embedding_dir]
        self.nerf_coarse = NeRF()
        self.models = [self.nerf_coarse]
        if hparams.N_importance > 0:
            self.nerf_fine = NeRF()
            self.models += [self.nerf_fine]
        self.train_dataset = train_dataset
        self.val_dataset = val_dataset
        self.white_back = getattr(train_dataset, 'white_back', getattr(hparams, 'white_back', False))
        self.fused_train_step = getattr(hparams, 'fused_train_step', True)
        self.fuse_adam = False

    @property
    def hp(self):
        return self.hparams_

    def decode_batch(self, batch):
        return batch['rays'], batch['rgbs']

    def forward(self, rays):
        B = rays.shape[0]
        hp = self.hp
        results = defaultdict(list)
        for i in range(0, B, hp.chunk):
            rendered = render_rays(self.models, self.embeddings, rays[i:i + hp.chunk], hp.N_samples, hp.use_disp,
                                   hp.perturb, hp.noise_std, hp.N_importance, hp.chunk, self.white_back)
            for k, v in rendered.items():
                results[k] += [v]
        for k, v in results.items():
            results[k] = torch.cat(v, 0) if len(v) > 1 else v[0]
        return results

    def configure_optimizers(self):
        hp = self.hp
        eps = 1e-8
        params = [p for m in self.models for p in m.parameters()]
        name = getattr(hp, 'optimizer', 'adam')
        wd = getattr(hp, 'weight_decay', 0)
        if name == 'adam':
            if params[0].is_cuda and getattr(hp, 'flat_optimizer', True):
                from .optim import FlatAdam
                self.optimizer = FlatAdam(self.models, lr=hp.lr, eps=eps, weight_decay=wd)
            else:
                self.optimizer = torch.optim.Adam(params, lr=hp.lr, eps=eps, weight_decay=wd, fused=params[0].is_cuda)
        elif name == 'sgd':
            self.optimizer = torch.optim.SGD(params, lr=hp.lr, momentum=getattr(hp, 'momentum', 0.9), weight_decay=wd)
        elif name in ('radam', 'ranger'):
            from .optim import FlatRAdam, FlatRanger
            self.optimizer = (FlatRAdam if name == 'radam' else FlatRanger)(self.models, lr=hp.lr, eps=eps, weight_decay=wd)
        else:
            raise ValueError('optimizer not recognized!')

        sched = getattr(hp, 'lr_scheduler', 'steplr')
        if sched == 'steplr':
            scheduler = torch.optim.lr_scheduler.MultiStepLR(self.optimizer, milestones=list(getattr(hp, 'decay_step', [20])),
                                                             gamma=getattr(hp, 'decay_gamma', 0.1))
        elif sched == 'cosine':
            scheduler = torch.optim.lr_scheduler.CosineAnnealingLR(self.optimizer, T_max=hp.num_epochs, eta_min=eps)
        elif sched == 'poly':
            n_ep, pexp = hp.num_epochs, getattr(hp, 'poly_exp', 0.9)
            scheduler = torch.optim.lr_scheduler.LambdaLR(self.optimizer, lambda epoch: (1 - epoch / n_ep) ** pexp)
        else:
            raise ValueError('scheduler not recognized!')
        if getattr(hp, 'warmup_epochs', 0) > 0 and name not in ('radam', 'ranger'):
            from .schedulers import GradualWarmupScheduler
            scheduler = GradualWarmupScheduler(self.optimizer, multiplier=getattr(hp, 'warmup_multiplier', 1.0),
                                               total_epoch=hp.warmup_epochs, after_scheduler=scheduler)
        return [self.optimizer], [scheduler]

    def training_step(self, batch, batch_nb):
        log = {'lr': get_learning_rate(self.optimizer)}
        rays, rgbs = self.decode_batch(batch)
        if self._fused_step_ok(rays):
            from .models.train_step import render_rays_train
            hp = self.hp
            adam = self.optimizer if (self.fuse_adam and type(self.optimizer).__name__ == 'FlatAdam'
                                      and self._fused_adam_ok()) else None
            draws = batch.get('draws') if isinstance(batch, dict) else None
            packed = batch.get('packed') if isinstance(batch, dict) else None
            results, loss, out3 = render_rays_train(self.models, self.embeddings, rays, rgbs, hp.N_samples, hp.use_disp, hp.perturb,
                                                    hp.noise_std, hp.N_importance, self.white_back, adam=adam, draws=draws, packed=packed)
            self.loss.last = out3
            log['train/loss'] = loss
            psnr_ = out3[1]
        else:
            results = self(rays)
            log['train/loss'] = loss = self.loss(results, rgbs)
            if getattr(self.loss, 'last', None) is not None:
                psnr_ = self.loss.last[1]
            else:
                typ = 'fine' if 'rgb_fine' in results else 'coarse'
                with torch.no_grad():
                    psnr_ = psnr(results[f'rgb_{typ}'], rgbs)
        log['train/psnr'] = psnr_
        return {'loss': loss, 'progress_bar': {'train_psnr': psnr_}, 'log': log}

    def _fused_adam_ok(self):
        import torch.distributed as dist
        return not (dist.is_available() and dist.is_initialized() and dist.get_world_size() > 1)

    def _fused_step_ok(self, rays):
        if not (self.fused_train_step and torch.is_grad_enabled() and rays.is_cuda and rays.dim() == 2
                and 0 < rays.shape[0] <= self.hp.chunk):
            return False
        from .models.train_step import fusable
        return fusable(self.models, self.embeddings, self.loss)

    def validation_panel(self, results, rgbs, H, W):
        from .visualization import visualize_depth
        typ = 'fine' if 'rgb_fine' in results else 'coarse'
        img = results[f'rgb_{typ}'].view(H, W, 3).permute(2, 0, 1)
        img_gt = rgbs.view(H, W, 3).permute(2, 0, 1)
        depth = visualize_depth(results[f'depth_{typ}'].view(H, W))
        return torch.stack([img_gt, img, depth])

    def validation_step(self, batch, batch_nb):
        rays, rgbs = self.decode_batch(batch)
        rays, rgbs = rays.squeeze(), rgbs.squeeze()
        results = self(rays)
        log = {'val_loss': self.loss(results, rgbs)}
        typ = 'fine' if 'rgb_fine' in results else 'coarse'
        if batch_nb == 0 and getattr(self, 'logger', None) is not None:
            W, H = self.hp.img_wh
            self.logger.experiment.add_images('val/GT_pred_depth', self.validation_panel(results, rgbs, H, W),
                                              getattr(self, 'global_step', 0))
        log['val_psnr'] = psnr(results[f'rgb_{typ}'], rgbs)
        return log

    def validation_epoch_end(self, outputs):
        mean_loss = torch.stack([x['val_loss'] for x in outputs]).mean()
        mean_psnr = torch.stack([x['val_psnr'] for x in outputs]).mean()
        return {'progress_bar': {'val_loss': mean_loss, 'val_psnr': mean_psnr},
                'log': {'val/loss': mean_loss, 'val/psnr': mean_psnr}}


def fit(system, batches, grad_sync=None, steps=None):
    (opt,), _ = system.configure_optimizers()
    losses = []
    for i, batch in enumerate(batches):
        if steps is not None and i >= steps:
            break
        out = system.training_step(batch, i)
        opt.zero_grad(set_to_none=True)
        out['loss'].backward()
        if grad_sync is not None:
            grad_sync.sync()
        opt.step()
        losses.append(out['loss'].detach())
    return losses


class GraphedTrainStep:

    def __init__(self, system, optimizer, grad_sync=None, warmup=3, sync_in_graph=None, backend=None, batch_source=None):
        self.system, self.opt, self.grad_sync = system, optimizer, grad_sync
        self.batch_source = batch_source
        self._seed = None
        self.warmup = warmup
        if sync_in_graph is None:
            sync_in_graph = os.environ.get("NERFHIP_SYNC_IN_GRAPH", "1") != "0"
        self.sync_in_graph = bool(sync_in_graph)
        self.calls = 0
        self.graph = None
        self.graph_opt = None
        self.static_batch = None
        self.static_out = None
        self.captured_lr = None
        self.capture_fallback = None
        self._draw_state = None
        self.backend = backend if backend is not None else _HipGraphBackend()

    @staticmethod
    def _detached(out):
        def d(v):
            return v.detach() if torch.is_tensor(v) else ({k: d(x) for k, x in v.items()} if isinstance(v, dict) else v)
        return d(out)

    def _fwd_bwd(self, batch):
        if self.batch_source is not None:
            batch = self.batch_source()
        out = self.system.training_step(batch, self.calls)
        self.opt.zero_grad(set_to_none=True)
        if self._seed is None:
            from .ops import unit_seed
            self._seed = unit_seed(out['loss']) if out['loss'].is_cuda else torch.ones_like(out['loss'])
        out['loss'].backward(self._seed)
        return self._detached(out)

    def _eager(self, batch):
        out = self._fwd_bwd(batch)
        if self.grad_sync is not None:
            self.grad_sync.sync()
        self.opt.step()
        return out

    def _two_graphs(self):
        return self.grad_sync is not None and not self.sync_in_graph

    def _set_hooks(self, on):
        if self.grad_sync is not None and hasattr(self.grad_sync, "hooks_enabled"):
            self.grad_sync.hooks_enabled = on

    def _arm_draws(self):
        p = next(iter(self.system.parameters()), None)
        if p is None or not p.is_cuda:
            return
        from .draws import GraphDrawState
        if self._draw_state is None:
            self._draw_state = GraphDrawState(p.device)
        self._draw_state.arm()

    def _capture_with_draws(self, fn, **kw):
        if self._draw_state is None:
            return self.backend.capture(fn, **kw)
        from .draws import capturing
        with capturing(self._draw_state):
            return self.backend.capture(fn, **kw)

    def _capture(self, batch):
        self.static_batch = {k: (v.clone() if torch.is_tensor(v) else {kk: vv.clone() for kk, vv in v.items()})
                             for k, v in batch.items() if torch.is_tensor(v) or isinstance(v, dict)} if batch is not None else None
        self.captured_lr = get_learning_rate(self.opt)
        self._arm_draws()
        self.static_out = None
        self.graph_opt = None
        if not self._two_graphs():
            err = None
            try:
                self.graph, self.static_out = self._capture_with_draws(lambda: self._eager(self.static_batch))
            except Exception as e:
                if self.grad_sync is None:
                    raise
                err = e
            failed = err is not None
            if self.grad_sync is not None and hasattr(self.grad_sync, "agree_any"):
                failed = self.grad_sync.agree_any(failed)
            if failed:
                import warnings
                warnings.warn("GraphedTrainStep: capturing the step with its all-reduces inside failed (%r); falling back to two "
                              "graphs with the collectives issued eagerly in between" % (err,))
                self.capture_fallback = repr(err) if err is not None else "another rank's capture failed"
                self.sync_in_graph = False
                self.graph = None
                getattr(self.grad_sync, "_inflight", {}).clear()
                self._arm_draws()
        if self._two_graphs():
            self._set_hooks(False)
            try:
                self.graph, self.static_out = self._capture_with_draws(lambda: self._fwd_bwd(self.static_batch))
                self.graph_opt, _ = self.backend.capture(self.opt.step, share_pool_with=self.graph)
            finally:
                self._set_hooks(True)

    def __call__(self, batch=None):
        if (batch is None) != (self.batch_source is not None):
            raise ValueError("pass a batch, or construct the stepper with a batch_source (not both)")
        self.calls += 1
        if self.calls <= self.warmup:
            return self.backend.on_side_stream(self._eager, batch)
        if (self.graph is None or get_learning_rate(self.opt) != self.captured_lr
                or (batch is not None and any(torch.is_tensor(batch[k]) and batch[k].shape != self.static_batch[k].shape for k in batch))):
            self._capture(batch)
        elif batch is not None:
            for k, v in batch.items():
                if torch.is_tensor(v):
                    self.static_batch[k].copy_(v, non_blocking=True)
                elif isinstance(v, dict):
                    for kk, vv in v.items():
                        self.static_batch[k][kk].copy_(vv, non_blocking=True)
        ds = self._draw_state
        if ds is not None and ds.increment:
            ds.before_replay()
        self.graph.replay()
        if ds is not None:
            ds.after_replay()
        if self.graph_opt is not None:
            self.grad_sync.sync()
            self.graph_opt.replay()
        return self.static_out


class _HipGraphBackend:

    def __init__(self, keep_graph=False):
        self.stream = torch.cuda.Stream()
        self.keep_graph = keep_graph

    def on_side_stream(self, fn, *args):
        self.stream.wait_stream(torch.cuda.current_stream())
        with torch.cuda.stream(self.stream):
            out = fn(*args)
        torch.cuda.current_stream().wait_stream(self.stream)
        return out

    def capture(self, fn, share_pool_with=None):
        graph = torch.cuda.CUDAGraph(keep_graph=True) if self.keep_graph else torch.cuda.CUDAGraph()
        torch.cuda.synchronize()
        kw = {"pool": share_pool_with.pool()} if share_pool_with is not None else {}
        with torch.cuda.graph(graph, stream=self.stream, capture_error_mode="thread_local", **kw):
            out = fn()
        return graph, out


def graph_node_count(graph):
    import ctypes
    try:
        raw = graph.raw_cuda_graph()
        hip = ctypes.CDLL("libamdhip64.so")
        n = ctypes.c_size_t(0)
        if hip.hipGraphGetNodes(ctypes.c_void_p(raw), None, ctypes.byref(n)) != 0:
            return None
        return int(n.value)
    except Exception:
        return None
```

Before: 1.099 million.

## Move MSE/PSNR loss reduction from render tail into backward reduce kernel

Removes the last-block ticket and atomic-load MSE/PSNR tail from the training render kernel, which frees its LDS and drops the per-block atomic and vmcnt wait. In the train-step runner the loss is deferred: the reduce kernel in the weight-gradient backward gets one extra block column that computes MSE/PSNR. When the loss is not deferred, a separate mse_psnr launch runs after the render. This trades a serialising tail in the forward kernel for one more block in an existing launch, but out3 is now only written during backward.

```diff
diff --git a/include/nerfhip.h b/include/nerfhip.h
--- a/include/nerfhip.h
+++ b/include/nerfhip.h
@@ -142,6 +142,19 @@
                                void* dw_workspace, float* const* grad_w_host, float* const* grad_b_host, int accumulate, int dtype,
                                int phases, const float* g_scale, const nerfhip_adam_fused* adam, const nerfhip_enc_source* enc,
                                nerfhip_stream_t stream);
+
+typedef struct nerfhip_loss_fold {
+    const float* rgb_coarse;
+    const float* rgb_fine;
+    const float* target;
+    int64_t n;
+    float* out3;
+} nerfhip_loss_fold;
+int nerfhip_mlp_bwd_multi_loss(int n_models, const float* const* g_out_host, const float* const* out_host, const int64_t* n_host,
+                               const void* const* packed_bwd_host, const void* const* acts_host, void* const* dys_host,
+                               void* dw_workspace, float* const* grad_w_host, float* const* grad_b_host, int accumulate, int dtype,
+                               int phases, const float* g_scale, const nerfhip_adam_fused* adam, const nerfhip_enc_source* enc,
+                               const nerfhip_loss_fold* loss, nerfhip_stream_t stream);
 
 int nerfhip_mlp_dx_embedded(const void* dys, int64_t n, const float* w_xyz1, const float* w_xyz5, const float* w_dir,
                             float* gx, int64_t gx_stride, int dtype, nerfhip_stream_t stream);
diff --git a/nerf_pl_amd/_lib.py b/nerf_pl_amd/_lib.py
--- a/nerf_pl_amd/_lib.py
+++ b/nerf_pl_amd/_lib.py
@@ -97,6 +97,10 @@
                                    ctypes.POINTER(_c_void_p), ctypes.POINTER(_c_void_p), ctypes.POINTER(_c_void_p), _c_void_p,
                                    ctypes.POINTER(_c_void_p), ctypes.POINTER(_c_void_p), _int, _int, _int, _c_void_p, _c_void_p, _c_void_p,
                                    _c_void_p],
+    "nerfhip_mlp_bwd_multi_loss": [_int, ctypes.POINTER(_c_void_p), ctypes.POINTER(_c_void_p), ctypes.POINTER(_i64),
+                                   ctypes.POINTER(_c_void_p), ctypes.POINTER(_c_void_p), ctypes.POINTER(_c_void_p), _c_void_p,
+                                   ctypes.POINTER(_c_void_p), ctypes.POINTER(_c_void_p), _int, _int, _int, _c_void_p, _c_void_p, _c_void_p,
+                                   _c_void_p, _c_void_p],
     "nerfhip_linear_fwd": [_c_void_p, _i64, _c_void_p, _i64, _c_void_p, _c_void_p, _i64, _i64, _int, _int, _int, _int, _int, _c_void_p],
     "nerfhip_linear_bwd_input": [_c_void_p, _i64, _c_void_p, _i64, _int, _c_void_p, _i64, _c_void_p, _i64, _i64, _int, _int, _int,
                                  _int, _c_void_p],
@@ -169,6 +173,10 @@
     _fields_ = [("rays", _c_void_p * 2), ("z", _c_void_p * 2), ("S", _int * 2)]
 
 
+class LossFold(ctypes.Structure):
+    _fields_ = [("rgb_coarse", _c_void_p), ("rgb_fine", _c_void_p), ("target", _c_void_p), ("n", _i64), ("out3", _c_void_p)]
+
+
 DRAW_UNIFORM, DRAW_NORMAL, DRAW_RANDINT = 0, 1, 2
 
 _RESTYPES = {"nerfhip_error_string": ctypes.c_char_p, "nerfhip_torch_draw_increment": ctypes.c_uint64, "nerfhip_mlp_packed_bytes": ctypes.c_size_t,
diff --git a/nerf_pl_amd/csrc/mlp_bwd.hip b/nerf_pl_amd/csrc/mlp_bwd.hip
--- a/nerf_pl_amd/csrc/mlp_bwd.hip
+++ b/nerf_pl_amd/csrc/mlp_bwd.hip
@@ -68,6 +68,16 @@
                                           void* const* dys_host, void* dw_workspace, float* const* grad_w_host,
                                           float* const* grad_b_host, int accumulate, int dtype, int phases, const float* g_scale,
                                           const nerfhip_adam_fused* adam, const nerfhip_enc_source* enc, nerfhip_stream_t stream) {
+    return nerfhip_mlp_bwd_multi_loss(n_models, g_out_host, out_host, n_host, packed_bwd_host, acts_host, dys_host, dw_workspace, grad_w_host,
+                                      grad_b_host, accumulate, dtype, phases, g_scale, adam, enc, nullptr, stream);
+}
+
+extern "C" int nerfhip_mlp_bwd_multi_loss(int n_models, const float* const* g_out_host, const float* const* out_host,
+                                          const int64_t* n_host, const void* const* packed_bwd_host, const void* const* acts_host,
+                                          void* const* dys_host, void* dw_workspace, float* const* grad_w_host,
+                                          float* const* grad_b_host, int accumulate, int dtype, int phases, const float* g_scale,
+                                          const nerfhip_adam_fused* adam, const nerfhip_enc_source* enc, const nerfhip_loss_fold* loss,
+                                          nerfhip_stream_t stream) {
     NERFHIP_CHECK_ARG(n_models >= 1 && n_models <= nerfhip::kDwMaxModels);
     if (!valid_dtype(dtype)) return NERFHIP_E_UNSUPPORTED;
     bool regen[nerfhip::kDwMaxModels] = {false, false};
@@ -83,6 +93,11 @@
     }
     NERFHIP_CHECK_ARG(g_out_host && out_host && n_host && packed_bwd_host && acts_host && dys_host && grad_w_host && grad_b_host);
     NERFHIP_CHECK_ARG(!(adam && accumulate));
+    nerfhip::LossFold L = {nullptr, nullptr, nullptr, 0, nullptr};
+    if (loss) {
+        NERFHIP_CHECK_ARG(loss->rgb_coarse && loss->target && loss->out3 && loss->n > 0 && (phases & 4));
+        L.rgb_coarse = loss->rgb_coarse; L.rgb_fine = loss->rgb_fine; L.target = loss->target; L.n = loss->n; L.out3 = loss->out3;
+    }
     nerfhip::GradTable G;
     nerfhip::DwJobTable jt;
     for (int m = 0; m < n_models; ++m) {
@@ -144,7 +159,7 @@
 #endif
     }
     if (do_reduce) {
-        nerfhip::launch_reduce(dtype == NERFHIP_BF16_F8, jt, (const float*)dw_workspace, G, fold_scratch, accumulate, A, s);
+        nerfhip::launch_reduce(dtype == NERFHIP_BF16_F8, jt, (const float*)dw_workspace, G, fold_scratch, accumulate, A, L, s);
         nerfhip::launch_fold(F, (const float*)fold_scratch, n_models, accumulate, A, s);
     }
     return nerfhip_launch_status();
diff --git a/nerf_pl_amd/csrc/mlp_bwd_dw.h b/nerf_pl_amd/csrc/mlp_bwd_dw.h
--- a/nerf_pl_amd/csrc/mlp_bwd_dw.h
+++ b/nerf_pl_amd/csrc/mlp_bwd_dw.h
@@ -49,6 +49,14 @@
     float lr, beta1, beta2, eps, wd;
 };
 
+struct LossFold {
+    const float* rgb_coarse;
+    const float* rgb_fine;
+    const float* target;
+    int64_t n;
+    float* out3;
+};
+
 struct FoldArgs {
     const float* image[kDwMaxModels];
     float* gw_final[kDwMaxModels];
@@ -59,7 +67,7 @@
 void launch_dw(int prec, const DwJobTable& jt, float* slabs, int nwg, hipStream_t s);
 void launch_dw_f8(const DwJobTable& jt, float* slabs, int nwg, hipStream_t s);
 void launch_reduce(bool f8, const DwJobTable& jt, const float* slabs, const GradTable& G, float* fold_scratch, int accumulate,
-                   const AdamFused& A, hipStream_t s);
+                   const AdamFused& A, const LossFold& L, hipStream_t s);
 void launch_fold(const FoldArgs& F, const float* fold_scratch, int n_models, int accumulate, const AdamFused& A, hipStream_t s);
 #if NERFHIP_DW_PROBE
 int read_dw_probe(unsigned* host_dst, int n_words);
diff --git a/nerf_pl_amd/csrc/mlp_bwd_reduce.hip b/nerf_pl_amd/csrc/mlp_bwd_reduce.hip
--- a/nerf_pl_amd/csrc/mlp_bwd_reduce.hip
+++ b/nerf_pl_amd/csrc/mlp_bwd_reduce.hip
@@ -1,5 +1,6 @@
 #include "mlp_device.h"
 #include "adam_math.h"
+#include "loss_math.h"
 #include "mlp_bwd_dw.h"
 
 namespace nerfhip {
@@ -20,7 +21,7 @@
 
 template <bool F8>
 __global__ __launch_bounds__(256) void mlp_bwd_reduce_kernel(DwJobTable jobs, const float* __restrict__ slabs, GradTable G,
-                                                              float* __restrict__ fold_scratch, int accumulate, AdamFused A) {
+                                                              float* __restrict__ fold_scratch, int accumulate, AdamFused A, LossFold L) {
     const int jid = blockIdx.y;
     const DwJob jb = jobs.job[jid];
     const int model = jid / kNumDwJobs;
@@ -35,7 +36,15 @@
     AdamCoef ac;
     if (A.state) ac = adam_coef(A.state[0] + 1.0f, A.lr, A.beta1, A.beta2);
     const GradEmit emit{A, ac, accumulate, model};
-    if (ot < n_ot && xt == kDwMaxXTiles) {
+    if (tile == 8 * (kDwMaxXTiles + 1)) {
+        if (jid == 0) {
+            __shared__ float red[2][16];
+            const float* __restrict__ img_c = L.rgb_coarse;
+            const float* __restrict__ img_f = L.rgb_fine;
+            mse_psnr_block<4>([&](int64_t i) { return img_c[i]; }, [&](int64_t i) { return img_f[i]; }, img_f != nullptr, L.target, L.n,
+                              L.out3, nullptr, nullptr, red);
+        }
+    } else if (ot < n_ot && xt == kDwMaxXTiles) {
         const int m = threadIdx.x;
         if (m < 32) {
             float sacc = 0.f;
@@ -190,10 +199,10 @@
 }
 
 void launch_reduce(bool f8, const DwJobTable& jt, const float* slabs, const GradTable& G, float* fold_scratch, int accumulate,
-                   const AdamFused& A, hipStream_t s) {
-    const dim3 rgrid(8 * (kDwMaxXTiles + 1), (unsigned)jt.njobs);
-    if (f8) hipLaunchKernelGGL(mlp_bwd_reduce_kernel<true>, rgrid, dim3(256), 0, s, jt, slabs, G, fold_scratch, accumulate, A);
-    else hipLaunchKernelGGL(mlp_bwd_reduce_kernel<false>, rgrid, dim3(256), 0, s, jt, slabs, G, fold_scratch, accumulate, A);
+                   const AdamFused& A, const LossFold& L, hipStream_t s) {
+    const dim3 rgrid(8 * (kDwMaxXTiles + 1) + (L.out3 ? 1 : 0), (unsigned)jt.njobs);
+    if (f8) hipLaunchKernelGGL(mlp_bwd_reduce_kernel<true>, rgrid, dim3(256), 0, s, jt, slabs, G, fold_scratch, accumulate, A, L);
+    else hipLaunchKernelGGL(mlp_bwd_reduce_kernel<false>, rgrid, dim3(256), 0, s, jt, slabs, G, fold_scratch, accumulate, A, L);
 }
 void launch_fold(const FoldArgs& F, const float* fold_scratch, int n_models, int accumulate, const AdamFused& A, hipStream_t s) {
     hipLaunchKernelGGL(mlp_bwd_fold_kernel, dim3(kFoldBlocks, (unsigned)n_models), dim3(256), 0, s, F, fold_scratch, accumulate, A);
diff --git a/nerf_pl_amd/csrc/mlp_render.hip b/nerf_pl_amd/csrc/mlp_render.hip
--- a/nerf_pl_amd/csrc/mlp_render.hip
+++ b/nerf_pl_amd/csrc/mlp_render.hip
@@ -43,7 +43,7 @@
     NERFHIP_CHECK_ARG(a->noise_std == 0.0f || (a->noise_coarse && (!fine || a->noise_fine)));
     NERFHIP_CHECK_ARG(a->row_total == NERFHIP_ROW_TOTAL_EXACT || a->row_total == NERFHIP_ROW_TOTAL_ATEN);
     if (train)
-        NERFHIP_CHECK_ARG(a->target && a->rgb_coarse && a->depth_coarse && a->g_raw_coarse && a->save_coarse && a->out3 && a->ticket &&
+        NERFHIP_CHECK_ARG(a->target && a->rgb_coarse && a->depth_coarse && a->g_raw_coarse && a->save_coarse &&
                           (!fine || (a->g_raw_fine && a->save_fine)));
     uintptr_t lines = (uintptr_t)a->z_coarse | (uintptr_t)a->raw_coarse | (uintptr_t)a->z_fine | (uintptr_t)a->raw_fine;
     if (train) lines |= (uintptr_t)a->g_raw_coarse | (uintptr_t)a->g_raw_fine;
@@ -84,7 +84,12 @@
     const int rc = render_check(args, dtype, true);
     if (rc) return rc;
     const unsigned groups = (unsigned)(args->B / kRenderRays);
-    if (dtype == NERFHIP_F32) return launch_render_variant<NERFHIP_F32, 1>(*args, groups, (hipStream_t)stream);
-    if (dtype == NERFHIP_BF16_F8) return launch_render_variant<NERFHIP_BF16, 2>(*args, groups, (hipStream_t)stream);
-    return launch_render_variant<NERFHIP_BF16, 1>(*args, groups, (hipStream_t)stream);
+    int st;
+    if (dtype == NERFHIP_F32) st = launch_render_variant<NERFHIP_F32, 1>(*args, groups, (hipStream_t)stream);
+    else if (dtype == NERFHIP_BF16_F8) st = launch_render_variant<NERFHIP_BF16, 2>(*args, groups, (hipStream_t)stream);
+    else st = launch_render_variant<NERFHIP_BF16, 1>(*args, groups, (hipStream_t)stream);
+    if (st == 0 && args->out3)
+        st = nerfhip_mse_psnr(args->rgb_coarse, args->N_i > 0 ? args->rgb_fine : nullptr, args->target, 3 * args->B, args->out3, nullptr,
+                              nullptr, stream);
+    return st;
 }
diff --git a/nerf_pl_amd/csrc/mlp_render_kernel.h b/nerf_pl_amd/csrc/mlp_render_kernel.h
--- a/nerf_pl_amd/csrc/mlp_render_kernel.h
+++ b/nerf_pl_amd/csrc/mlp_render_kernel.h
@@ -78,8 +78,6 @@
     constexpr int FSV = TT ? 0 : SV;
     constexpr int NW = PrecTraits<PREC>::NW, PTS = 32 * NW, R = kRenderRays;
     __shared__ __attribute__((aligned(1024))) char lds_all[FwdLds<PREC, TRAIN>::kBytes];
-    __shared__ float red[2][16];
-    __shared__ unsigned last_s;
     const int lane = threadIdx.x & 63;
     const int wave = __builtin_amdgcn_readfirstlane((int)(threadIdx.x >> 6));
     float* const tail_lds = reinterpret_cast<float*>(lds_all + FwdLds<PREC, TRAIN>::kRingOff);
@@ -115,33 +113,6 @@
     }
     render_wg_sync();
     render_tail<TRAIN, NW, TT>(nf > 0, false, tail_lds, wave, lane);
-
-    if constexpr (TRAIN) {
-        const RenderArgsP a = render_args();
-        unsigned* const ticket = a->ticket;
-        asm volatile("s_waitcnt vmcnt(0)" ::: "memory");
-        __syncthreads();
-        if (threadIdx.x == 0) {
-            const unsigned prev = __hip_atomic_fetch_add(ticket, 1u, __ATOMIC_RELAXED, __HIP_MEMORY_SCOPE_AGENT);
-            last_s = (prev == gridDim.x - 1) ? 1u : 0u;
-            if (prev == gridDim.x - 1) __hip_atomic_store(ticket, 0u, __ATOMIC_RELAXED, __HIP_MEMORY_SCOPE_AGENT);
-        }
-        __syncthreads();
-        if (!last_s) return;
-        __builtin_amdgcn_fence(__ATOMIC_ACQUIRE, "agent");
-        const float* img_c = a->rgb_coarse;
-        const float* img_f = a->rgb_fine;
-        const float* target = a->target;
-        float* out3 = a->out3;
-        const int64_t n3 = 3 * a->B;
-        auto fresh_c = [&](int64_t i) { return __hip_atomic_load(img_c + i, __ATOMIC_RELAXED, __HIP_MEMORY_SCOPE_AGENT); };
-        auto fresh_f = [&](int64_t i) { return __hip_atomic_load(img_f + i, __ATOMIC_RELAXED, __HIP_MEMORY_SCOPE_AGENT); };
-        constexpr int Q = 1024 / (NW * 64);
-        if (nf > 0)
-            mse_psnr_block<Q>(fresh_c, fresh_f, true, target, n3, out3, nullptr, nullptr, red);
-        else
-            mse_psnr_block<Q>(fresh_c, [&](int64_t i) { return 0.0f; }, false, target, n3, out3, nullptr, nullptr, red);
-    }
 }
 
 template <int PREC, int SV>
diff --git a/nerf_pl_amd/models/train_step.py b/nerf_pl_amd/models/train_step.py
--- a/nerf_pl_amd/models/train_step.py
+++ b/nerf_pl_amd/models/train_step.py
@@ -54,7 +54,7 @@
 class _TrainRender(torch.autograd.Function):
     @staticmethod
     def forward(ctx, cfg, rays, rgbs, *params):
-        models, S, use_disp, perturb, noise_std, N, white_back, adam, draws, packed = cfg
+        models, S, use_disp, perturb, noise_std, N, white_back, adam, draws, packed, defer_loss = cfg
         rays = rays.float().contiguous()
         rgbs = rgbs.float().contiguous()
         B = rays.shape[0]
@@ -74,12 +74,15 @@
         packs = [m.train_buffers(dtype, dev) for m in models] if fresh else ops.pack_models_train(models, dtype)
         gscale = float(np.float32(2.0) / np.float32(3 * B))
         acts_c = ops.alloc_acts(B * S, dtype, dev)
+        ctx.loss_fold = None
         if ops.render_supported(B, S, N, dtype):
             acts_f = ops.alloc_acts(B * (S + N), dtype, dev) if N > 0 else None
             regen = regen_enc_enabled() and ops.mlp_dtype_code(dtype) == ops.BF16 and S % 32 == 0 and (S + N) % 32 == 0
             o = ops.render_train_fwd(rays, rgbs, gscale, S, N, packs[0][0], packs[1][0] if N > 0 else None, dtype, acts_c, acts_f,
-                                     use_disp, perturb, perturb_rand, noise_c, noise_f, noise_std, white_back, u, regen_enc=regen)
+                                     use_disp, perturb, perturb_rand, noise_c, noise_f, noise_std, white_back, u, regen_enc=regen,
+                                     defer_loss=defer_loss)
             out3 = o["out3"]
+            ctx.loss_fold = o.get("loss_fold")
             outs = [o["rgb_coarse"], o["depth_coarse"], o["opacity_coarse"]]
             entries = [(o["g_raw_coarse"], o["raw_coarse"], packs[0][1], acts_c) + ((rays, o["z_coarse"]) if regen else ())]
             if N > 0:
@@ -99,9 +102,13 @@
     @staticmethod
     def backward(ctx, g_loss, *_unused):
         n_models = len(ctx.n_params)
+        loss_fold, ctx.loss_fold = getattr(ctx, "loss_fold", None), None
         if g_loss is None:
+            if loss_fold is not None:
+                ops.loss_fold_now(loss_fold)
             return (None, None, None) + (None,) * sum(ctx.n_params)
         entries = ctx.entries
+        lf = {} if loss_fold is None else {"loss_fold": loss_fold}
         g_scale = None if ops.is_unit_seed(g_loss) else g_loss.reshape(1).float().contiguous()
         models, dtype = ctx.models, ctx.dtype
         for m, serial in zip(models, ctx.serials):
@@ -109,14 +116,15 @@
         hooked = any(getattr(m, "_grad_ready_hook", None) is not None for m in models)
         joint_hook = getattr(models[0], "_grads_ready_hook", None) if hooked else None
         if hooked and joint_hook is not None and all(getattr(m, "_grads_ready_hook", None) == joint_hook for m in models):
-            grads = ops.mlp_bwd_multi(entries, dtype, g_scale=g_scale)
+            grads = ops.mlp_bwd_multi(entries, dtype, g_scale=g_scale, **lf)
             for m, g in zip(models, grads):
                 m._flat_grad = g[2]
             joint_hook(models, [g[2] for g in grads])
         elif hooked:
             grads = []
             for m, entry in zip(models, entries):
-                ((gw, gb, flat),) = ops.mlp_bwd_multi([entry], dtype, g_scale=g_scale)
+                ((gw, gb, flat),) = ops.mlp_bwd_multi([entry], dtype, g_scale=g_scale, **lf)
+                lf = {}
                 m._flat_grad = flat
                 m._grad_ready_hook(m, flat)
                 grads.append((gw, gb, flat))
@@ -124,7 +132,7 @@
             if ctx.adam is not None and any(p.grad is not None for m in models for p in m.flat_params()):
                 ctx.adam = None
             adam = ctx.adam.handle(models) if ctx.adam is not None else None
-            grads = ops.mlp_bwd_multi(entries, dtype, adam=adam, g_scale=g_scale)
+            grads = ops.mlp_bwd_multi(entries, dtype, adam=adam, g_scale=g_scale, **lf)
             for m, g in zip(models, grads):
                 m._flat_grad = g[2]
             if ctx.adam is not None:
@@ -140,11 +148,11 @@
 
 
 def render_rays_train(models, embeddings, rays, rgbs, N_samples=64, use_disp=False, perturb=0, noise_std=1, N_importance=0,
-                      white_back=False, adam=None, draws=None, packed=None):
+                      white_back=False, adam=None, draws=None, packed=None, defer_loss=False):
     N = int(N_importance)
     use = list(models[:2]) if N > 0 else [models[0]]
     params = [p for m in use for p in m.flat_params()]
-    cfg = (use, int(N_samples), bool(use_disp), float(perturb), float(noise_std), N, bool(white_back), adam, draws, packed)
+    cfg = (use, int(N_samples), bool(use_disp), float(perturb), float(noise_std), N, bool(white_back), adam, draws, packed, bool(defer_loss))
     res = _TrainRender.apply(cfg, rays, rgbs, *params)
     loss, out3 = res[0], res[1]
     results = {'rgb_coarse': res[2], 'depth_coarse': res[3], 'opacity_coarse': res[4]}
diff --git a/nerf_pl_amd/ops.py b/nerf_pl_amd/ops.py
--- a/nerf_pl_amd/ops.py
+++ b/nerf_pl_amd/ops.py
@@ -532,7 +532,7 @@
 @device_guard
 def render_train_fwd(rays, target, grad_scale, n_samples, n_importance, packed_coarse, packed_fine, dtype, acts_coarse, acts_fine,
                      use_disp=False, perturb=0.0, perturb_rand=None, noise_coarse=None, noise_fine=None, noise_std=0.0,
-                     white_back=False, u=None, eps=1e-5, regen_enc=False):
+                     white_back=False, u=None, eps=1e-5, regen_enc=False, defer_loss=False):
     require_gpu(rays, target, perturb_rand, noise_coarse, noise_fine, u)
     rays, target = _c(rays), _c(target)
     B, S, N = rays.shape[0], int(n_samples), int(n_importance)
@@ -547,11 +547,12 @@
     bufs["out3"] = torch.empty(3, device=dev, dtype=torch.float32)
     a.g_raw_coarse = bufs["g_raw_coarse"].data_ptr()
     a.g_raw_fine = bufs["g_raw_fine"].data_ptr() if N > 0 else None
-    a.out3 = bufs["out3"].data_ptr()
+    a.out3 = None if defer_loss else bufs["out3"].data_ptr()
+    if defer_loss:
+        bufs["loss_fold"] = (bufs["rgb_coarse"], bufs["rgb_fine"] if N > 0 else None, target, bufs["out3"])
     a.save_coarse = acts_coarse.data_ptr()
     a.save_fine = acts_fine.data_ptr() if N > 0 else None
     a.target, a.grad_scale = target.data_ptr(), float(grad_scale)
-    a.ticket = _ticket(dev).data_ptr()
     a.regen_enc = int(bool(regen_enc) and mlp_dtype_code(dtype) == BF16)
     check(_lib.load().nerfhip_render_train_fwd(ctypes.addressof(a), mlp_dtype_code(dtype), stream_ptr()), "nerfhip_render_train_fwd")
     return bufs
@@ -644,7 +645,15 @@
     return bufs
 
 
-def mlp_bwd_multi(entries, dtype, adam=None, phases=7, workspace=None, g_scale=None):
+def loss_fold_now(loss_fold):
+    rgb_c, rgb_f, target, out3 = loss_fold
+    with torch.cuda.device(out3.device):
+        check(_lib.load().nerfhip_mse_psnr(ptr(rgb_c), ptr(rgb_f), ptr(target), target.numel(), ptr(out3), None, None, stream_ptr()),
+              "nerfhip_mse_psnr")
+    return out3
+
+
+def mlp_bwd_multi(entries, dtype, adam=None, phases=7, workspace=None, g_scale=None, loss_fold=None):
     code = mlp_dtype_code(dtype)
     lib = _lib.load()
     M = len(entries)
@@ -694,9 +703,20 @@
                 adam.grad_flat[m] = grads[m][2].data_ptr()
         if g_scale is not None:
             require_gpu(g_scale)
-        check(lib.nerfhip_mlp_bwd_multi_rays(M, G, O, n_arr, PB, AC, DY, ptr(ws), GW, GB, 0, code, int(phases), ptr(g_scale),
+        lf = None
+        if loss_fold is not None:
+            rgb_c, rgb_f, target, out3 = loss_fold
+            require_gpu(rgb_c, rgb_f, target, out3)
+            if (rgb_c.numel() != target.numel() or (rgb_f is not None and rgb_f.numel() != target.numel()) or out3.numel() != 3
+                    or any(t.dtype != torch.float32 or not t.is_contiguous() for t in (rgb_c, target, out3) + ((rgb_f,) if rgb_f is not None else ()))):
+                raise ValueError("mlp_bwd_multi: loss_fold = (rgb_coarse, rgb_fine | None, target, out3) contiguous fp32, images of one size")
+            lf = _lib.LossFold()
+            lf.rgb_coarse, lf.target, lf.n, lf.out3 = rgb_c.data_ptr(), target.data_ptr(), target.numel(), out3.data_ptr()
+            lf.rgb_fine = rgb_f.data_ptr() if rgb_f is not None else None
+        check(lib.nerfhip_mlp_bwd_multi_loss(M, G, O, n_arr, PB, AC, DY, ptr(ws), GW, GB, 0, code, int(phases), ptr(g_scale),
                                              ctypes.addressof(adam) if adam is not None else None,
-                                             ctypes.addressof(enc) if enc is not None else None, stream_ptr()), "nerfhip_mlp_bwd_multi_rays")
+                                             ctypes.addressof(enc) if enc is not None else None,
+                                             ctypes.addressof(lf) if lf is not None else None, stream_ptr()), "nerfhip_mlp_bwd_multi_loss")
     return grads
 
 
diff --git a/nerf_pl_amd/system.py b/nerf_pl_amd/system.py
--- a/nerf_pl_amd/system.py
+++ b/nerf_pl_amd/system.py
@@ -42,6 +42,7 @@
         self.white_back = getattr(train_dataset, 'white_back', getattr(hparams, 'white_back', False))
         self.fused_train_step = getattr(hparams, 'fused_train_step', True)
         self.fuse_adam = False
+        self.loss_in_backward = False
 
     @property
     def hp(self):
@@ -111,7 +112,8 @@
             draws = batch.get('draws') if isinstance(batch, dict) else None
             packed = batch.get('packed') if isinstance(batch, dict) else None
             results, loss, out3 = render_rays_train(self.models, self.embeddings, rays, rgbs, hp.N_samples, hp.use_disp, hp.perturb,
-                                                    hp.noise_std, hp.N_importance, self.white_back, adam=adam, draws=draws, packed=packed)
+                                                    hp.noise_std, hp.N_importance, self.white_back, adam=adam, draws=draws, packed=packed,
+                                                    defer_loss=self.loss_in_backward)
             self.loss.last = out3
             log['train/loss'] = loss
             psnr_ = out3[1]
@@ -211,7 +213,12 @@
     def _fwd_bwd(self, batch):
         if self.batch_source is not None:
             batch = self.batch_source()
-        out = self.system.training_step(batch, self.calls)
+        prev = getattr(self.system, "loss_in_backward", False)
+        self.system.loss_in_backward = True
+        try:
+            out = self.system.training_step(batch, self.calls)
+        finally:
+            self.system.loss_in_backward = prev
         self.opt.zero_grad(set_to_none=True)
         if self._seed is None:
             from .ops import unit_seed
```

New measurement: 1.104 million, median of 4. About the same (+0.4%).
